# basilevh/tcow

Measured on AMD Instinct MI355X. Metric: train clips/sec (T=30, 240x320), higher is better.
Workload: dtype bf16; 1 GPU; TCOW Seeker train step: T=30 240x320 patch16, 12-layer divided space-time ViT (D=768), num_queries=3, causal_attention=1, 1 clip/GPU; clips_per_gpu=1, num_queries=3, parallelism=dp1, optimizer=AdamW lr 1e-4, clip 0.3

## Files before the change

include/tcow_hip.h:

```cpp
#ifndef TCOW_HIP_H
#define TCOW_HIP_H

#ifdef __cplusplus
extern "C" {
#endif

#define TCOW_OK 0
#define TCOW_ERR_INVALID_ARG (-1)
#define TCOW_ERR_LAUNCH (-2)
#define TCOW_ERR_UNSUPPORTED (-3)

#define TCOW_F32 0
#define TCOW_BF16 1
#define TCOW_F32X3 2

#define TCOW_ACT_NONE 0
#define TCOW_ACT_GELU 1
#define TCOW_ACT_DGELU 2
#define TCOW_ACT_GELU_DSAVE 3
#define TCOW_ACT_MUL_AUX 4

#define TCOW_ABI_VERSION 11
int tcow_version(void);
const char* tcow_last_error(void);

typedef struct {
    int M, N, K;
    int dtype;
    const void* A; long lda;
    const void* W; long ldw;
    void* C; long ldc; int out_f32;
    const float* bias;
    const float* row_scale;
    const float* resid; long ldr;
    int act;
    void* aux; long ldaux;
    int tile;
    const float* bias2;
    const float* row_scale2;
} tcow_gemm_args;
int tcow_gemm_nt(void* stream, const tcow_gemm_args* args);

int tcow_prof_gemm_begin(int max_launches);
int tcow_prof_gemm_end(double* total_ms, double* total_flops, long* launches);
int tcow_prof_attn_begin(int max_launches);
int tcow_prof_attn_end(double* ms4, double* flops4, double* bytes4, long* launches4);

long tcow_gemm_tn_workspace_bytes(int M, int N, int K);
int tcow_gemm_tn(void* stream, int dtype, int M, int N, int K, const void* dY, long ldy, const void* X,
                 long ldx, float* dW, long lddw, float* bias_grad, int accumulate, void* workspace,
                 long workspace_bytes);

typedef struct {
    int M, N, K;
    const void* dY; long ldy;
    const void* X; long ldx;
    float* dW; long lddw;
    float* bias_grad;
    int accumulate;
} tcow_tn_problem;
long tcow_gemm_tn_grouped_workspace_bytes(int dtype, int n, const tcow_tn_problem* problems);
int tcow_gemm_tn_grouped(void* stream, int dtype, int n, const tcow_tn_problem* problems, void* workspace, long workspace_bytes);
int tcow_gemm_tn_group_max(void);

typedef struct {
    int M, N, K;
    const float* A; long sai, sak;
    const float* B; long sbj, sbk;
    float* C; long ldc;
    int accumulate;
} tcow_sgemm;
int tcow_sgemm_x3_batched(void* stream, int n, const tcow_sgemm* problems);

int tcow_layernorm_fwd(void* stream, int dtype, int rows, int D, const float* x, long ldx, const float* gamma,
                       const float* beta, float eps, void* y, long ldy, float* mean, float* rstd);
long tcow_layernorm_bwd_workspace_bytes(int D);
int tcow_layernorm_bwd(void* stream, int dtype, int rows, int D, const void* dy, long lddy, const float* x, long ldx,
                       const float* mean, const float* rstd, const float* gamma, const float* dres, long lddres,
                       float* dx, long lddx, float* dgamma, float* dbeta, int accumulate, void* workspace,
                       long workspace_bytes, void* dx_cast, long lddx_cast, const float* cast_row_scale,
                       const float* colsum_row_scale, float* colsum_out);
typedef struct {
    const float* part; int parts, D;
    float* dgamma; float* dbeta; float* colsum_out;
    int accumulate;
} tcow_ln_fold_job;
int tcow_layernorm_bwd_parts(int rows, int with_colsum);
int tcow_layernorm_fold(void* stream, int n, const tcow_ln_fold_job* jobs);

typedef struct {
    int B, T, S;
    int D, heads;
    int causal;
    int dtype;
} tcow_attn_shape;
int tcow_attn_temporal_fwd(void* stream, const tcow_attn_shape* shape, const void* qkv, void* out, float* lse);
int tcow_attn_spatial_fwd(void* stream, const tcow_attn_shape* shape, const void* qkv, void* out, float* lse);
long tcow_attn_bwd_workspace_bytes(const tcow_attn_shape* shape);
int tcow_attn_temporal_bwd(void* stream, const tcow_attn_shape* shape, const void* qkv, const void* out,
                           const void* dout, const float* lse, void* dqkv, void* workspace, long workspace_bytes);
int tcow_attn_spatial_bwd(void* stream, const tcow_attn_shape* shape, const void* qkv, const void* out,
                          const void* dout, const float* lse, void* dqkv, void* workspace, long workspace_bytes);

#define TCOW_STREAM_MAX_FRAMES 1024
int tcow_attn_temporal_cached_fwd(void* stream, const tcow_attn_shape* chunk, int T_total, const int* t0_dev, const void* qkv, void* k_cache,
                                  void* v_cache, void* out);
int tcow_cls_stream(void* stream, int B, int c, int S, int D, float* x, float* cls_cache, const int* t0_dev);

int tcow_im2col(void* stream, int dtype, int B, int T, int H, int W, int P, const float* rgb, const float* query,
                int pretrained_norm, void* out);
int tcow_im2col_channels(void* stream, int dtype, int B, int T, int H, int W, int P, int C, const float* src,
                         int normalise, void* out);
int tcow_gather_frames(void* stream, int elem_bytes, int C, int Tv, int H, int W, int Tc, int h, int w, const void* src,
                       const int* frame_idx, const int* src_y, const int* src_x, void* out);
int tcow_resize_aa(void* stream, int C, int Tv, int H, int W, int Tc, int hc, int wc, int oh, int ow, const float* src, const int* frame_idx,
                   const int* ys, const int* xs, const int* ymin, const int* ysize, const float* wy, int ky, const int* xmin, const int* xsize,
                   const float* wx, int kx, float* out);

long tcow_photometric_workspace_bytes(int Tc);
int tcow_photometric(void* stream, int Tv, int H, int W, int Tc, int y0, int x0, int h, int w, const float* src, const int* frame_idx, int n_ops,
                     const int* ops, float brightness, float contrast, float saturation, float hue, int blur, const float* taps, int gray,
                     float* workspace, long workspace_bytes, float* out);

int tcow_embed_fwd(void* stream, int B, int T, int S, int D, float* x, const float* cls, const float* pos,
                   const float* time_embed);
int tcow_embed_bwd(void* stream, int B, int T, int S, int D, const float* g, float* dpos, float* dtime,
                   int accumulate);
int tcow_cls_merge(void* stream, int B, int T, int S, int D, float* x, int mode, int backward);
int tcow_cls_merge_bwd_cast(void* stream, int dtype, int B, int T, int S, int D, float* x, int mode, void* cast_out, long ldc,
                            const float* cast_scale);

int tcow_unpatchify_pool_fwd(void* stream, int dtype, int BT, int Hp, int Wp, int P, int C, int st, const void* pm,
                             float* pooled);
int tcow_unpatchify_pool_bwd(void* stream, int dtype, int BT, int Hp, int Wp, int P, int C, int st,
                             const float* dpooled, void* dpm);
int tcow_upsample_fwd(void* stream, int B, int T, int C, int h, int w, int st, int bilinear, const float* pooled,
                      float* out);
int tcow_upsample_bwd(void* stream, int B, int T, int C, int h, int w, int st, int bilinear, const float* dout,
                      float* dpooled);
#define TCOW_AMAX_SLOTS 64
int tcow_upsample_bwd_amax(void* stream, int B, int T, int C, int h, int w, int st, const float* dout, float* dpooled,
                           unsigned* amax_bits, int n_slots);
int tcow_flags_fwd(void* stream, int BT, int S, int D, int F, const float* x, const float* Wf, const float* bf,
                   float* flags);

int tcow_scale_unless_one(void* stream, float* x, long n, const float* scale);
int tcow_scale_cast(void* stream, int dtype, long rows, int D, const float* src, long ld_src, const float* row_scale,
                    void* dst, long ld_dst);
int tcow_droppath_rows(void* stream, int depth, int B, int T, int S, const float* u, const float* keep_p, const float* mask0, float* out);
int tcow_cast_transpose(void* stream, int dtype, int N, int K, const float* W, void* Wc, void* Wt);
long tcow_cast_desc_bytes(void);
int tcow_cast_transpose_batched(void* stream, int dtype, const void* table, int n, int total_tiles);

long tcow_adamw_chunk_bytes(void);
int tcow_adamw_clip_step(void* stream, const void* chunks, int n_chunks, float lr, float beta1, float beta2, float eps,
                         float weight_decay, int step, float max_norm, float* scratch);
int tcow_adamw_clip_step_scaled(void* stream, const void* chunks, int n_chunks, float lr, float beta1, float beta2, float eps,
                                float weight_decay, int step, float max_norm, float* scratch, const float* grad_inv_scale);
long tcow_adamw_tile_bytes(void);
int tcow_adamw_clip_step_cast(void* stream, const void* chunks, int n_chunks, const void* flat_chunks, int n_flat, const void* tiles, int n_tiles, float lr, float beta1,
                              float beta2, float eps, float weight_decay, int step, float max_norm, float* scratch, const float* grad_inv_scale);

typedef struct {
    long n_frames, frame_len, frames_per_seq;
    const float* logits;  long logits_seq_stride;
    const float* target;  long target_seq_stride;
    const float* pixel_w;
    const float* frame_w;
    int weighted_aot;
    float aot_loss;
    double topk_frac;
    float loss_weight;
    float* loss;
    float* total;
    float* dlogits;  long dlogits_seq_stride;
    void* ws;  size_t ws_bytes;
    int focal;
} tcow_mask_loss_args;
size_t tcow_mask_loss_workspace_bytes(long n_frames, long frame_len);
size_t tcow_mask_loss_workspace_bytes_for(long n_frames, long frame_len, double topk_frac, float aot_loss);
int tcow_mask_loss(void* stream, const tcow_mask_loss_args* args);
int tcow_mask_loss_batch(void* stream, const tcow_mask_loss_args* args, int n);

int tcow_iou_counts(void* stream, const float* logits, const float* target, long n_frames, long frame_len, int* counts);

int tcow_build_masks(void* stream, int B, int Q, int M, int T, long HW, int query_time, const unsigned char* segm,
                     const unsigned char* div_segm, const int* query_idx, const int* front_idx, const int* cont_idx,
                     float* query_mask, float* target_mask, unsigned char* snitch_occl_by_ptr, int* counts);

int tcow_build_query_masks(void* stream, int B, int Q, int K, int M, int T, long HW, int query_time, const unsigned char* segm,
                           const unsigned char* div_segm, const float* occl_fracs, const float* dag, const long long* sel, float front_thres,
                           float front_half_thres, float outer_thres, float occluded_weight, float zero_weight, float has_weight, int* idx_ws,
                           unsigned char* ids, float* flags, float* sel_occl_fracs, float* frame_w, float* query_mask, float* target_mask,
                           unsigned char* snitch_occl_by_ptr, int* counts);

int tcow_iou_means(void* stream, const int* counts, int n_seq, int C, int T, float* mean, int* count);

size_t tcow_snitch_weights_workspace_bytes(long n_frames, int H, int W);
int tcow_snitch_weights(void* stream, long n_seq, int T, int H, int W, const float* target_ch0, long target_seq_stride,
                        const unsigned char* snitch_occl_by_ptr, const float* frame_w, const int* pos_count, int class_balancing,
                        float hard_negative_factor, float* weights, void* ws, size_t ws_bytes);

#ifdef __cplusplus
}
#endif
#endif
```

tcow_amd/_lib.py:

```python
import ctypes
import os

_HERE = os.path.dirname(os.path.abspath(__file__))
LIB_PATH = os.environ.get('TCOW_LIB') or os.path.join(_HERE, 'libtcow_hip.so')
LIB_PATH_FP16 = os.path.join(_HERE, 'libtcow_hip_fp16.so')

TCOW_F32, TCOW_BF16, TCOW_F32X3 = 0, 1, 2
ACT_NONE, ACT_GELU, ACT_DGELU, ACT_GELU_DSAVE, ACT_MUL_AUX = 0, 1, 2, 3, 4


class TcowError(RuntimeError):
    """Raised when a libtcow_hip entry point returns a non-zero status (message from tcow_last_error)."""


class AttnShape(ctypes.Structure):
    _fields_ = [('B', ctypes.c_int), ('T', ctypes.c_int), ('S', ctypes.c_int), ('D', ctypes.c_int),
                ('heads', ctypes.c_int), ('causal', ctypes.c_int), ('dtype', ctypes.c_int)]


class GemmArgs(ctypes.Structure):
    _fields_ = [('M', ctypes.c_int), ('N', ctypes.c_int), ('K', ctypes.c_int), ('dtype', ctypes.c_int),
                ('A', ctypes.c_void_p), ('lda', ctypes.c_long), ('W', ctypes.c_void_p), ('ldw', ctypes.c_long),
                ('C', ctypes.c_void_p), ('ldc', ctypes.c_long), ('out_f32', ctypes.c_int),
                ('bias', ctypes.c_void_p), ('row_scale', ctypes.c_void_p), ('resid', ctypes.c_void_p),
                ('ldr', ctypes.c_long), ('act', ctypes.c_int), ('aux', ctypes.c_void_p), ('ldaux', ctypes.c_long), ('tile', ctypes.c_int),
                ('bias2', ctypes.c_void_p), ('row_scale2', ctypes.c_void_p)]


class SGemm(ctypes.Structure):
    _fields_ = [('M', ctypes.c_int), ('N', ctypes.c_int), ('K', ctypes.c_int),
                ('A', ctypes.c_void_p), ('sai', ctypes.c_long), ('sak', ctypes.c_long),
                ('B', ctypes.c_void_p), ('sbj', ctypes.c_long), ('sbk', ctypes.c_long),
                ('C', ctypes.c_void_p), ('ldc', ctypes.c_long), ('accumulate', ctypes.c_int)]


class TnProblem(ctypes.Structure):
    _fields_ = [('M', ctypes.c_int), ('N', ctypes.c_int), ('K', ctypes.c_int),
                ('dY', ctypes.c_void_p), ('ldy', ctypes.c_long), ('X', ctypes.c_void_p), ('ldx', ctypes.c_long),
                ('dW', ctypes.c_void_p), ('lddw', ctypes.c_long), ('bias_grad', ctypes.c_void_p), ('accumulate', ctypes.c_int)]


class LnFoldJob(ctypes.Structure):
    _fields_ = [('part', ctypes.c_void_p), ('parts', ctypes.c_int), ('D', ctypes.c_int), ('dgamma', ctypes.c_void_p), ('dbeta', ctypes.c_void_p),
                ('colsum_out', ctypes.c_void_p), ('accumulate', ctypes.c_int)]


class MaskLossArgs(ctypes.Structure):
    _fields_ = [('n_frames', ctypes.c_long), ('frame_len', ctypes.c_long), ('frames_per_seq', ctypes.c_long),
                ('logits', ctypes.c_void_p), ('logits_seq_stride', ctypes.c_long),
                ('target', ctypes.c_void_p), ('target_seq_stride', ctypes.c_long),
                ('pixel_w', ctypes.c_void_p), ('frame_w', ctypes.c_void_p),
                ('weighted_aot', ctypes.c_int), ('aot_loss', ctypes.c_float), ('topk_frac', ctypes.c_double),
                ('loss_weight', ctypes.c_float), ('loss', ctypes.c_void_p), ('total', ctypes.c_void_p),
                ('dlogits', ctypes.c_void_p), ('dlogits_seq_stride', ctypes.c_long),
                ('ws', ctypes.c_void_p), ('ws_bytes', ctypes.c_size_t), ('focal', ctypes.c_int)]


_libs = {}

_vp, _i, _l, _f = ctypes.c_void_p, ctypes.c_int, ctypes.c_long, ctypes.c_float
_ash = ctypes.POINTER(AttnShape)
SIGNATURES = {
    'tcow_version': (_i, []),
    'tcow_last_error': (ctypes.c_char_p, []),
    'tcow_gemm_nt': (_i, [_vp, ctypes.POINTER(GemmArgs)]),
    'tcow_prof_gemm_begin': (_i, [_i]),
    'tcow_prof_gemm_end': (_i, [ctypes.POINTER(ctypes.c_double), ctypes.POINTER(ctypes.c_double), ctypes.POINTER(ctypes.c_long)]),
    'tcow_prof_attn_begin': (_i, [_i]),
    'tcow_prof_attn_end': (_i, [_vp, _vp, _vp, _vp]),
    'tcow_gemm_tn_workspace_bytes': (_l, [_i, _i, _i]),
    'tcow_gemm_tn': (_i, [_vp, _i, _i, _i, _i, _vp, _l, _vp, _l, _vp, _l, _vp, _i, _vp, _l]),
    'tcow_gemm_tn_grouped_workspace_bytes': (_l, [_i, _i, _vp]),
    'tcow_gemm_tn_grouped': (_i, [_vp, _i, _i, _vp, _vp, _l]),
    'tcow_gemm_tn_group_max': (_i, []),
    'tcow_sgemm_x3_batched': (_i, [_vp, _i, _vp]),
    'tcow_layernorm_fwd': (_i, [_vp, _i, _i, _i, _vp, _l, _vp, _vp, _f, _vp, _l, _vp, _vp]),
    'tcow_layernorm_bwd_workspace_bytes': (_l, [_i]),
    'tcow_layernorm_bwd': (_i, [_vp, _i, _i, _i, _vp, _l, _vp, _l, _vp, _vp, _vp, _vp, _l, _vp, _l, _vp, _vp, _i, _vp, _l, _vp, _l, _vp, _vp, _vp]),
    'tcow_layernorm_bwd_parts': (_i, [_i, _i]),
    'tcow_layernorm_fold': (_i, [_vp, _i, _vp]),
    'tcow_attn_temporal_fwd': (_i, [_vp, _ash, _vp, _vp, _vp]),
    'tcow_attn_spatial_fwd': (_i, [_vp, _ash, _vp, _vp, _vp]),
    'tcow_attn_bwd_workspace_bytes': (_l, [_ash]),
    'tcow_attn_temporal_bwd': (_i, [_vp, _ash, _vp, _vp, _vp, _vp, _vp, _vp, _l]),
    'tcow_attn_spatial_bwd': (_i, [_vp, _ash, _vp, _vp, _vp, _vp, _vp, _vp, _l]),
    'tcow_attn_temporal_cached_fwd': (_i, [_vp, _ash, _i, _vp, _vp, _vp, _vp, _vp]),
    'tcow_cls_stream': (_i, [_vp, _i, _i, _i, _i, _vp, _vp, _vp]),
    'tcow_im2col': (_i, [_vp, _i, _i, _i, _i, _i, _i, _vp, _vp, _i, _vp]),
    'tcow_gather_frames': (_i, [_vp, _i, _i, _i, _i, _i, _i, _i, _i, _vp, _vp, _vp, _vp, _vp]),
    'tcow_resize_aa': (_i, [_vp, _i, _i, _i, _i, _i, _i, _i, _i, _i, _vp, _vp, _vp, _vp, _vp, _vp, _vp, _i, _vp, _vp, _vp, _i, _vp]),
    'tcow_photometric_workspace_bytes': (_l, [_i]),
    'tcow_photometric': (_i, [_vp, _i, _i, _i, _i, _i, _i, _i, _i, _vp, _vp, _i, ctypes.POINTER(ctypes.c_int), _f, _f, _f, _f, _i, ctypes.POINTER(ctypes.c_float), _i,
                         _vp, _l, _vp]),
    'tcow_im2col_channels': (_i, [_vp, _i, _i, _i, _i, _i, _i, _i, _vp, _i, _vp]),
    'tcow_embed_fwd': (_i, [_vp, _i, _i, _i, _i, _vp, _vp, _vp, _vp]),
    'tcow_embed_bwd': (_i, [_vp, _i, _i, _i, _i, _vp, _vp, _vp, _i]),
    'tcow_cls_merge': (_i, [_vp, _i, _i, _i, _i, _vp, _i, _i]),
    'tcow_cls_merge_bwd_cast': (_i, [_vp, _i, _i, _i, _i, _i, _vp, _i, _vp, _l, _vp]),
    'tcow_unpatchify_pool_fwd': (_i, [_vp, _i, _i, _i, _i, _i, _i, _i, _vp, _vp]),
    'tcow_unpatchify_pool_bwd': (_i, [_vp, _i, _i, _i, _i, _i, _i, _i, _vp, _vp]),
    'tcow_upsample_fwd': (_i, [_vp, _i, _i, _i, _i, _i, _i, _i, _vp, _vp]),
    'tcow_upsample_bwd': (_i, [_vp, _i, _i, _i, _i, _i, _i, _i, _vp, _vp]),
    'tcow_upsample_bwd_amax': (_i, [_vp, _i, _i, _i, _i, _i, _i, _vp, _vp, _vp, _i]),
    'tcow_flags_fwd': (_i, [_vp, _i, _i, _i, _i, _vp, _vp, _vp, _vp]),
    'tcow_droppath_rows': (_i, [_vp, _i, _i, _i, _i, _vp, _vp, _vp, _vp]),
    'tcow_scale_cast': (_i, [_vp, _i, _l, _i, _vp, _l, _vp, _vp, _l]),
    'tcow_scale_unless_one': (_i, [_vp, _vp, _l, _vp]),
    'tcow_cast_transpose': (_i, [_vp, _i, _i, _i, _vp, _vp, _vp]),
    'tcow_cast_desc_bytes': (_l, []),
    'tcow_cast_transpose_batched': (_i, [_vp, _i, _vp, _i, _i]),
    'tcow_adamw_chunk_bytes': (_l, []),
    'tcow_adamw_clip_step': (_i, [_vp, _vp, _i, _f, _f, _f, _f, _f, _i, _f, _vp]),
    'tcow_adamw_clip_step_scaled': (_i, [_vp, _vp, _i, _f, _f, _f, _f, _f, _i, _f, _vp, _vp]),
    'tcow_adamw_tile_bytes': (_l, []),
    'tcow_adamw_clip_step_cast': (_i, [_vp, _vp, _i, _vp, _i, _vp, _i, _f, _f, _f, _f, _f, _i, _f, _vp, _vp]),
    'tcow_mask_loss_workspace_bytes': (ctypes.c_size_t, [_l, _l]),
    'tcow_mask_loss_workspace_bytes_for': (ctypes.c_size_t, [_l, _l, ctypes.c_double, _f]),
    'tcow_mask_loss': (_i, [_vp, ctypes.POINTER(MaskLossArgs)]),
    'tcow_mask_loss_batch': (_i, [_vp, ctypes.POINTER(MaskLossArgs), _i]),
    'tcow_iou_counts': (_i, [_vp, _vp, _vp, _l, _l, _vp]),
    'tcow_build_masks': (_i, [_vp, _i, _i, _i, _i, _l, _i, _vp, _vp, _vp, _vp, _vp, _vp, _vp, _vp, _vp]),
    'tcow_build_query_masks': (_i, [_vp, _i, _i, _i, _i, _i, _l, _i, _vp, _vp, _vp, _vp, _vp, _f, _f, _f, _f, _f, _f, _vp, _vp, _vp, _vp, _vp, _vp, _vp, _vp, _vp]),
    'tcow_iou_means': (_i, [_vp, _vp, _i, _i, _i, _vp, _vp]),
    'tcow_snitch_weights_workspace_bytes': (ctypes.c_size_t, [_l, _i, _i]),
    'tcow_snitch_weights': (_i, [_vp, _l, _i, _i, _i, _vp, _l, _vp, _vp, _vp, _i, _f, _vp, _vp, ctypes.c_size_t]),
}


ABI_VERSION = 11


def _declare(L, tolerant=False):
    for name, (res, args) in SIGNATURES.items():
        if tolerant and not hasattr(L, name):
            continue
        fn = getattr(L, name)
        fn.restype = res
        fn.argtypes = args



def lib(fmt='bf16'):
    L = _libs.get(fmt)
    if L is None:
        path = LIB_PATH if fmt == 'bf16' else LIB_PATH_FP16
        if not os.path.exists(path):
            raise TcowError(f'{path} not found: build it with `make` (or __graft_entry__.build()); '
                            'the Seeker HIP path has no fallback')
        import torch
        L = ctypes.CDLL(path)
        L.tcow_last_error.restype = ctypes.c_char_p
        L.tcow_version.restype = ctypes.c_int
        if L.tcow_version() != ABI_VERSION and not (fmt == 'bf16' and os.environ.get('TCOW_LIB')):
            raise TcowError(f'{path} reports ABI version {L.tcow_version()}, this host code was written against {ABI_VERSION} (include/tcow_hip.h): rebuild with `make`')
        _declare(L, tolerant=(fmt == 'bf16' and bool(os.environ.get('TCOW_LIB'))))
        _libs[fmt] = L
    return L


def check(rc, what='', L=None):
    if rc != 0:
        raise TcowError(f'{what} failed (status {rc}): {(L or lib()).tcow_last_error().decode()}')
```

tcow_amd/csrc/common.h:

```cpp
#pragma once
#include <hip/hip_runtime.h>
#include <stdint.h>

#include "../../include/tcow_hip.h"

#ifdef TCOW_FP16
typedef _Float16 tcow_h16;
#define TCOW_MFMA_32x32x16_H16 __builtin_amdgcn_mfma_f32_32x32x16_f16
#define TCOW_MFMA_32x32x16_H16_ASM "v_mfma_f32_32x32x16_f16"
#else
typedef __bf16 tcow_h16;
#define TCOW_MFMA_32x32x16_H16 __builtin_amdgcn_mfma_f32_32x32x16_bf16
#define TCOW_MFMA_32x32x16_H16_ASM "v_mfma_f32_32x32x16_bf16"
#endif
typedef __attribute__((ext_vector_type(8))) tcow_h16 bf16x8;
typedef __attribute__((ext_vector_type(4))) tcow_h16 bf16x4;
typedef __attribute__((ext_vector_type(2))) tcow_h16 bf16x2;
typedef __attribute__((ext_vector_type(16))) float f32x16;
typedef __attribute__((ext_vector_type(4))) float f32x4;
typedef __attribute__((ext_vector_type(2))) float f32x2;
typedef __attribute__((ext_vector_type(4))) short s16x4;
typedef uint16_t bf16_t;

#define LDS_PTR(T) __attribute__((address_space(3))) T*
#define GLB_PTR(T) __attribute__((address_space(1))) T*

void tcow_set_error(const char* fmt, ...);
#define TCOW_CHECK_ARG(cond, ...)                 \
    do {                                          \
        if (!(cond)) {                            \
            tcow_set_error(__VA_ARGS__);          \
            return TCOW_ERR_INVALID_ARG;          \
        }                                         \
    } while (0)
#define TCOW_CHECK_LAUNCH()                                                        \
    do {                                                                           \
        hipError_t e__ = hipGetLastError();                                        \
        if (e__ != hipSuccess) {                                                   \
            tcow_set_error("%s: launch failed: %s", __func__, hipGetErrorString(e__)); \
            return TCOW_ERR_LAUNCH;                                                \
        }                                                                          \
    } while (0)

__device__ __forceinline__ float bf2f(bf16_t h) {
#ifdef TCOW_FP16
    return (float)__builtin_bit_cast(_Float16, h);
#else
    return __builtin_bit_cast(float, ((uint32_t)h) << 16);
#endif
}
__device__ __forceinline__ bf16_t f2bf(float f) { return __builtin_bit_cast(bf16_t, (tcow_h16)f); }
__device__ __forceinline__ uint32_t pack_bf2(float lo, float hi) {
    f32x2 v = {lo, hi};
    bf16x2 b = __builtin_convertvector(v, bf16x2);
    return __builtin_bit_cast(uint32_t, b);
}
#ifdef TCOW_FP16
__device__ __forceinline__ float bflo(uint32_t u) { return (float)__builtin_bit_cast(_Float16, (uint16_t)(u & 0xffffu)); }
__device__ __forceinline__ float bfhi(uint32_t u) { return (float)__builtin_bit_cast(_Float16, (uint16_t)(u >> 16)); }
#else
__device__ __forceinline__ float bflo(uint32_t u) { return __builtin_bit_cast(float, u << 16); }
__device__ __forceinline__ float bfhi(uint32_t u) { return __builtin_bit_cast(float, u & 0xffff0000u); }
#endif

template <typename T> struct Elem;
template <> struct Elem<float> {
    static __device__ __forceinline__ float ld(const float* p) { return *p; }
    static __device__ __forceinline__ void st(float* p, float v) { *p = v; }
};
template <> struct Elem<bf16_t> {
    static __device__ __forceinline__ float ld(const bf16_t* p) { return bf2f(*p); }
    static __device__ __forceinline__ void st(bf16_t* p, float v) { *p = f2bf(v); }
};

__device__ __forceinline__ float4 ld4(const float* p) { return *reinterpret_cast<const float4*>(p); }
__device__ __forceinline__ float4 ld4(const bf16_t* p) {
    uint2 u = *reinterpret_cast<const uint2*>(p);
    return make_float4(bflo(u.x), bfhi(u.x), bflo(u.y), bfhi(u.y));
}
__device__ __forceinline__ void st4(float* p, float4 v) { *reinterpret_cast<float4*>(p) = v; }
__device__ __forceinline__ void st4(bf16_t* p, float4 v) {
    uint2 u; u.x = pack_bf2(v.x, v.y); u.y = pack_bf2(v.z, v.w);
    *reinterpret_cast<uint2*>(p) = u;
}

typedef uint32_t tcow_u32x4 __attribute__((ext_vector_type(4)));
template <bool NT> __device__ __forceinline__ void st16c(void* p, uint4 w) {
    if constexpr (NT) __builtin_nontemporal_store((tcow_u32x4){w.x, w.y, w.z, w.w}, reinterpret_cast<tcow_u32x4*>(p)); else *reinterpret_cast<uint4*>(p) = w;
}
template <bool NT> __device__ __forceinline__ uint4 ld16c(const void* p) {
    if constexpr (NT) { const tcow_u32x4 v = __builtin_nontemporal_load(reinterpret_cast<const tcow_u32x4*>(p)); return make_uint4(v[0], v[1], v[2], v[3]); } else return *reinterpret_cast<const uint4*>(p);
}

__device__ __forceinline__ float gelu_erf(float x) { return 0.5f * x * (1.0f + erff(x * 0.70710678118654752440f)); }
__device__ __forceinline__ float gelu_erf_grad(float x) {
    const float cdf = 0.5f * (1.0f + erff(x * 0.70710678118654752440f));
    const float pdf = 0.39894228040143267794f * __expf(-0.5f * x * x);
    return cdf + x * pdf;
}

__device__ __forceinline__ float wave_sum(float v) {
#pragma unroll
    for (int o = 32; o > 0; o >>= 1) v += __shfl_xor(v, o, 64);
    return v;
}
__device__ __forceinline__ float wave_max(float v) {
#pragma unroll
    for (int o = 32; o > 0; o >>= 1) v = fmaxf(v, __shfl_xor(v, o, 64));
    return v;
}

__host__ __device__ __forceinline__ constexpr int crow32(int r, int hi) { return (r & 3) + 8 * (r >> 2) + 4 * hi; }

void tcow_ensure_lds(const void* kernel, int bytes);

static inline int cdiv(long a, long b) { return (int)((a + b - 1) / b); }
```

tcow_amd/csrc/elementwise.hip:

```cpp
#include "common.h"

namespace {

template <typename T>
__global__ void im2col_kernel(int B, int T_, int H, int W, int P, int Crgb, int Cq, const float* __restrict__ rgb, const float* __restrict__ qm, int norm,
                              T* __restrict__ out) {
    const int Hp = H / P, Wp = W / P, N = Hp * Wp, S = N + 1, C = Crgb + Cq;
    const int Kc = C * P * P, q4 = Kc / 4;
    const long total = (long)B * T_ * S * q4;
    for (long i = blockIdx.x * (long)blockDim.x + threadIdx.x; i < total; i += (long)gridDim.x * blockDim.x) {
        const long row = i / q4; const int k = (int)(i - row * q4) * 4;
        const int s = (int)(row % S); const long bt = row / S; const int t = (int)(bt % T_); const int b = (int)(bt / T_);
        float4 v = make_float4(0.f, 0.f, 0.f, 0.f);
        if (s > 0) {
            const int n = s - 1, hp = n / Wp, wp = n - hp * Wp;
            const int c = k / (P * P), rem = k - c * P * P, py = rem / P, px = rem - py * P;
            const int y = hp * P + py, x = wp * P + px;
            if (c < Crgb) {
                v = ld4(rgb + ((((size_t)b * Crgb + c) * T_ + t) * H + y) * W + x);
                if (norm) { v.x = (v.x - 0.45f) / 0.225f; v.y = (v.y - 0.45f) / 0.225f; v.z = (v.z - 0.45f) / 0.225f; v.w = (v.w - 0.45f) / 0.225f; }
            } else {
                v = ld4(qm + ((((size_t)b * Cq + (c - Crgb)) * T_ + t) * H + y) * W + x);
            }
        }
        st4(out + row * Kc + k, v);
    }
}

template <typename T>
__global__ void gather_frames_kernel(int C, int Tv, int H, int W, int Tc, int h, int w, const T* __restrict__ src, const int* __restrict__ frame_idx,
                                     const int* __restrict__ src_y, const int* __restrict__ src_x, T* __restrict__ out) {
    const long total = (long)C * Tc * h * w;
    for (long i = blockIdx.x * (long)blockDim.x + threadIdx.x; i < total; i += (long)gridDim.x * blockDim.x) {
        const int x = (int)(i % w); long r = i / w; const int y = (int)(r % h); r /= h; const int t = (int)(r % Tc); const int c = (int)(r / Tc);
        out[i] = src[(((size_t)c * Tv + frame_idx[t]) * H + src_y[y]) * W + src_x[x]];
    }
}

__global__ void resize_aa_kernel(int C, int Tv, int H, int W, int Tc, int oh, int ow, const float* __restrict__ src, const int* __restrict__ frame_idx,
                                 const int* __restrict__ ys, const int* __restrict__ xs, const int* __restrict__ ymin, const int* __restrict__ ysize,
                                 const float* __restrict__ wy, int ky, const int* __restrict__ xmin, const int* __restrict__ xsize, const float* __restrict__ wx, int kx,
                                 float* __restrict__ out) {
    const long total = (long)C * Tc * oh * ow;
    for (long i = blockIdx.x * (long)blockDim.x + threadIdx.x; i < total; i += (long)gridDim.x * blockDim.x) {
        const int X = (int)(i % ow); long r = i / ow; const int Y = (int)(r % oh); r /= oh; const int t = (int)(r % Tc); const int c = (int)(r / Tc);
        const float* plane = src + ((size_t)c * Tv + frame_idx[t]) * H * W;
        const int x0 = xmin[X], nx = xsize[X], y0 = ymin[Y], ny = ysize[Y];
        float acc = 0.f;
        for (int j = 0; j < ny; ++j) {
            const float* row = plane + (size_t)ys[y0 + j] * W;
            float h = 0.f;
            for (int k = 0; k < nx; ++k) h += wx[(size_t)X * kx + k] * row[xs[x0 + k]];
            acc += wy[(size_t)Y * ky + j] * h;
        }
        out[i] = acc;
    }
}

__global__ void embed_fwd_kernel(int B, int T_, int S, int D, float* __restrict__ x, const float* __restrict__ cls, const float* __restrict__ pos,
                                 const float* __restrict__ time) {
    const int d4 = D / 4;
    const long total = (long)B * T_ * S * d4;
    for (long i = blockIdx.x * (long)blockDim.x + threadIdx.x; i < total; i += (long)gridDim.x * blockDim.x) {
        const long row = i / d4; const int c = (int)(i - row * d4) * 4;
        const int s = (int)(row % S); const int t = (int)((row / S) % T_);
        const float4 p = ld4(pos + (size_t)s * D + c);
        float4 o;
        if (s == 0) { const float4 cv = ld4(cls + c); o = make_float4(cv.x + p.x, cv.y + p.y, cv.z + p.z, cv.w + p.w); }
        else {
            const float4 v = ld4(x + row * D + c), te = ld4(time + (size_t)t * D + c);
            o = make_float4(v.x + p.x + te.x, v.y + p.y + te.y, v.z + p.z + te.z, v.w + p.w + te.w);
        }
        st4(x + row * D + c, o);
    }
}
__global__ __launch_bounds__(256) void embed_bwd_pos_kernel(int B, int T_, int S, int D, const float* __restrict__ g, float* __restrict__ dpos, int accumulate) {
    __shared__ float4 red[256];
    const int d4 = D / 4, s = blockIdx.x, q = blockIdx.y * 64 + (threadIdx.x & 63), part = threadIdx.x >> 6, BT = B * T_;
    float4 a = make_float4(0.f, 0.f, 0.f, 0.f);
    if (q < d4) {
        const float* src = g + (size_t)s * D + q * 4;
        const size_t fs = (size_t)S * D;
        int bt = part;
        for (; bt + 20 < BT; bt += 24) {
            float4 v[6];
#pragma unroll
            for (int u = 0; u < 6; ++u) v[u] = ld4(src + (size_t)(bt + 4 * u) * fs);
#pragma unroll
            for (int u = 0; u < 6; ++u) { a.x += v[u].x; a.y += v[u].y; a.z += v[u].z; a.w += v[u].w; }
        }
        for (; bt < BT; bt += 4) { const float4 v = ld4(src + (size_t)bt * fs); a.x += v.x; a.y += v.y; a.z += v.z; a.w += v.w; }
    }
    red[threadIdx.x] = a;
    __syncthreads();
    if (part == 0 && q < d4) {
#pragma unroll
        for (int p = 1; p < 4; ++p) { const float4 v = red[p * 64 + threadIdx.x]; a.x += v.x; a.y += v.y; a.z += v.z; a.w += v.w; }
        float* o = dpos + (size_t)s * D + q * 4;
        if (accumulate) { const float4 p = ld4(o); a.x += p.x; a.y += p.y; a.z += p.z; a.w += p.w; }
        st4(o, a);
    }
}
__global__ __launch_bounds__(256) void embed_bwd_time_kernel(int B, int T_, int S, int D, const float* __restrict__ g, float* __restrict__ dtime, int accumulate) {
    __shared__ float4 red[256];
    const int t = blockIdx.x, cq = blockIdx.y * 16 + (threadIdx.x & 15), part = threadIdx.x >> 4;
    const int d4 = D / 4;
    float4 a = make_float4(0.f, 0.f, 0.f, 0.f);
    if (cq < d4) {
        for (int b = 0; b < B; ++b)
            for (int s = 1 + part; s < S; s += 16) {
                const float4 v = ld4(g + (((size_t)b * T_ + t) * S + s) * D + cq * 4); a.x += v.x; a.y += v.y; a.z += v.z; a.w += v.w;
            }
    }
    red[threadIdx.x] = a;
    __syncthreads();
    if (part == 0 && cq < d4) {
        for (int p = 1; p < 16; ++p) { const float4 v = red[p * 16 + (threadIdx.x & 15)]; a.x += v.x; a.y += v.y; a.z += v.z; a.w += v.w; }
        float* o = dtime + (size_t)t * D + cq * 4;
        if (accumulate) { const float4 p = ld4(o); a.x += p.x; a.y += p.y; a.z += p.z; a.w += p.w; }
        st4(o, a);
    }
}

__device__ __forceinline__ float4 sum_frames(const float* base, size_t fs, int T_) {
    float4 a = make_float4(0.f, 0.f, 0.f, 0.f);
    for (int t0 = 0; t0 < T_; t0 += 8) {
        float4 v[8];
#pragma unroll
        for (int u = 0; u < 8; ++u) v[u] = t0 + u < T_ ? ld4(base + (t0 + u) * fs) : make_float4(0.f, 0.f, 0.f, 0.f);
#pragma unroll
        for (int u = 0; u < 8; ++u) { a.x += v[u].x; a.y += v[u].y; a.z += v[u].z; a.w += v[u].w; }
    }
    return a;
}
template <typename CT>
__global__ void cls_merge_kernel(int B, int T_, int S, int D, float* __restrict__ x, int mode, int backward, CT* __restrict__ cast_out, long ldc,
                                 const float* __restrict__ cast_scale) {
    const int d4 = D / 4;
    const long i = blockIdx.x * (long)blockDim.x + threadIdx.x;
    if (i >= (long)B * d4) return;
    const int b = (int)(i / d4), c = (int)(i - (long)b * d4) * 4;
    float* base = x + (size_t)b * T_ * S * D + c;
    const size_t fs = (size_t)S * D;
    if (!backward) {
        float4 a;
        if (mode == 1) a = ld4(base);
        else {
            a = sum_frames(base, fs, T_);
            const float inv = 1.0f / (float)T_; a.x *= inv; a.y *= inv; a.z *= inv; a.w *= inv;
        }
        for (int t = 0; t < T_; ++t) st4(base + t * fs, a);
    } else {
        float4 a = sum_frames(base, fs, T_);
        if (mode == 1) {
            st4(base, a);
            const float4 z = make_float4(0.f, 0.f, 0.f, 0.f);
            for (int t = 1; t < T_; ++t) st4(base + t * fs, z);
        } else {
            const float inv = 1.0f / (float)T_; a.x *= inv; a.y *= inv; a.z *= inv; a.w *= inv;
            for (int t = 0; t < T_; ++t) st4(base + t * fs, a);
        }
        if (cast_out) {
            for (int t0 = 0; t0 < T_; t0 += 8) {
                float cs[8];
#pragma unroll
                for (int u = 0; u < 8; ++u) cs[u] = (cast_scale && t0 + u < T_ && !(mode == 1 && t0 + u > 0)) ? cast_scale[((long)b * T_ + t0 + u) * S] : 1.0f;
#pragma unroll
                for (int u = 0; u < 8; ++u) {
                    const int t = t0 + u;
                    if (t < T_) {
                        const float4 v = (mode == 1 && t > 0) ? make_float4(0.f, 0.f, 0.f, 0.f) : make_float4(a.x * cs[u], a.y * cs[u], a.z * cs[u], a.w * cs[u]);
                        st4(cast_out + ((long)b * T_ + t) * S * ldc + c, v);
                    }
                }
            }
        }
    }
}

template <typename T>
__global__ void unpatchify_pool_fwd_kernel(int BT, int Hp, int Wp, int P, int C, int st, const T* __restrict__ pm, float* __restrict__ pooled) {
    const int S = Hp * Wp + 1, Ps = P / st, Ho = Hp * Ps, Wo = Wp * Ps, K = C * P * P;
    const long total = (long)BT * C * Ho * Wo;
    const float inv = 1.0f / (float)(st * st);
    for (long i = blockIdx.x * (long)blockDim.x + threadIdx.x; i < total; i += (long)gridDim.x * blockDim.x) {
        const int X = (int)(i % Wo); const int Y = (int)((i / Wo) % Ho); const int c = (int)((i / ((long)Wo * Ho)) % C); const long bt = i / ((long)Wo * Ho * C);
        const int hp = Y / Ps, py0 = (Y - hp * Ps) * st, wp = X / Ps, px0 = (X - wp * Ps) * st;
        const T* src = pm + ((size_t)bt * S + 1 + hp * Wp + wp) * K + (size_t)c * P * P;
        float a = 0.f;
        for (int dy = 0; dy < st; ++dy)
            for (int dx = 0; dx < st; ++dx) a += Elem<T>::ld(src + (py0 + dy) * P + px0 + dx);
        pooled[i] = a * inv;
    }
}
template <typename T>
__global__ __launch_bounds__(256) void unpatchify_pool4_fwd_kernel(int BT, int Hp, int Wp, int P, int C, const T* __restrict__ pm, float* __restrict__ pooled) {
    const int S = Hp * Wp + 1, Ps = P / 4, Ho = Hp * Ps, Wo = Wp * Ps, K = C * P * P, P8 = P / 8;
    const int per_tok = C * Ps * P8;
    const long total = (long)BT * (S - 1) * per_tok;
    for (long i = blockIdx.x * (long)blockDim.x + threadIdx.x; i < total; i += (long)gridDim.x * blockDim.x) {
        const int tok = (int)(i / per_tok), r = (int)(i - (long)tok * per_tok);
        const int piece = r % P8, yb = (r / P8) % Ps, c = r / (P8 * Ps);
        const int bt = tok / (S - 1), n = tok - bt * (S - 1), hp = n / Wp, wp = n - hp * Wp;
        const T* src = pm + ((size_t)bt * S + 1 + n) * K + (size_t)c * P * P + (4 * yb) * P + piece * 8;
        float a0 = 0.f, a1 = 0.f;
#pragma unroll
        for (int dy = 0; dy < 4; ++dy) {
            const float4 u = ld4(src + dy * P), v = ld4(src + dy * P + 4);
            a0 += (u.x + u.y) + (u.z + u.w); a1 += (v.x + v.y) + (v.z + v.w);
        }
        float* o = pooled + (((size_t)bt * C + c) * Ho + hp * Ps + yb) * Wo + wp * Ps + piece * 2;
        *reinterpret_cast<float2*>(o) = make_float2(a0 * 0.0625f, a1 * 0.0625f);
    }
}

template <typename T>
__global__ void unpatchify_pool_bwd_kernel(int BT, int Hp, int Wp, int P, int C, int st, const float* __restrict__ dpooled, T* __restrict__ dpm) {
    const int S = Hp * Wp + 1, Ps = P / st, Ho = Hp * Ps, Wo = Wp * Ps, K = C * P * P;
    const long total = (long)BT * S * K;
    const float inv = 1.0f / (float)(st * st);
    for (long i = blockIdx.x * (long)blockDim.x + threadIdx.x; i < total; i += (long)gridDim.x * blockDim.x) {
        const int k = (int)(i % K); const long row = i / K; const int s = (int)(row % S); const long bt = row / S;
        float v = 0.f;
        if (s > 0) {
            const int n = s - 1, hp = n / Wp, wp = n - hp * Wp;
            const int c = k / (P * P), rem = k - c * P * P, py = rem / P, px = rem - py * P;
            const int Y = hp * Ps + py / st, X = wp * Ps + px / st;
            v = dpooled[(((size_t)bt * C + c) * Ho + Y) * Wo + X] * inv;
        }
        Elem<T>::st(dpm + i, v);
    }
}

template <typename T>
__global__ __launch_bounds__(256) void unpatchify_pool_bwd8_kernel(int rows, int Hp, int Wp, int P, int C, int st, const float* __restrict__ dpooled, T* __restrict__ dpm) {
    const int S = Hp * Wp + 1, Ps = P / st, Ho = Hp * Ps, Wo = Wp * Ps, K = C * P * P, K8 = K >> 3;
    const float inv = 1.0f / (float)(st * st);
    const long total = (long)rows * K8;
    for (long i = blockIdx.x * (long)blockDim.x + threadIdx.x; i < total; i += (long)gridDim.x * blockDim.x) {
        const int row = (int)(i / K8), k = (int)(i - (long)row * K8) * 8;
        const int bt = row / S, s = row - bt * S;
        float v[8] = {0.f, 0.f, 0.f, 0.f, 0.f, 0.f, 0.f, 0.f};
        if (s > 0) {
            const int n = s - 1, hp = n / Wp, wp = n - hp * Wp;
            const int c = k / (P * P), rem = k - c * P * P, py = rem / P, px = rem - py * P;
            const float* src = dpooled + (((size_t)bt * C + c) * Ho + hp * Ps + py / st) * Wo + wp * Ps;
#pragma unroll
            for (int e = 0; e < 8; ++e) v[e] = src[(px + e) / st] * inv;
        }
        T* dst = dpm + (size_t)row * K + k;
        st4(dst, make_float4(v[0], v[1], v[2], v[3]));
        st4(dst + 4, make_float4(v[4], v[5], v[6], v[7]));
    }
}

__device__ __forceinline__ void bil_src(int dst, int in, int out, int& i0, int& i1, float& w0, float& w1) {
    const float scale = (out > 1) ? (float)(in - 1) / (float)(out - 1) : 0.f;
    const float src = scale * (float)dst;
    i0 = (int)src; if (i0 > in - 1) i0 = in - 1;
    i1 = i0 + ((i0 < in - 1) ? 1 : 0);
    w1 = src - (float)i0; w0 = 1.0f - w1;
}
__global__ void upsample_fwd_kernel(int B, int T_, int C, int h, int w, int st, int bilinear, const float* __restrict__ pooled, float* __restrict__ out) {
    const int H = h * st, W = w * st;
    const int f = blockIdx.y;
    const int t = f % T_, bc = f / T_, c = bc % C, b = bc / C;
    const float* src = pooled + (((size_t)(b * T_ + t)) * C + c) * h * w;
    float* dst = out + (size_t)f * H * W;
    const int Wq = (W + 3) / 4;
    for (int i = blockIdx.x * blockDim.x + threadIdx.x; i < H * Wq; i += gridDim.x * blockDim.x) {
        const int y = i / Wq, x0q = (i - y * Wq) * 4;
        float v[4];
        int y0, y1; float wy0, wy1;
        if (bilinear) bil_src(y, h, H, y0, y1, wy0, wy1);
#pragma unroll
        for (int e = 0; e < 4; ++e) {
            const int x = x0q + e < W ? x0q + e : W - 1;
            if (bilinear) {
                int x0, x1; float wx0, wx1;
                bil_src(x, w, W, x0, x1, wx0, wx1);
                v[e] = wy0 * (wx0 * src[y0 * w + x0] + wx1 * src[y0 * w + x1]) + wy1 * (wx0 * src[y1 * w + x0] + wx1 * src[y1 * w + x1]);
            } else {
                v[e] = src[(y / st) * w + (x / st)];
            }
        }
        float* o = dst + (size_t)y * W + x0q;
        if ((W & 3) == 0) st4(o, make_float4(v[0], v[1], v[2], v[3]));
        else for (int e = 0; e < 4 && x0q + e < W; ++e) o[e] = v[e];
    }
}
__global__ void upsample_bwd_kernel(int B, int T_, int C, int h, int w, int st, int bilinear, const float* __restrict__ dout, float* __restrict__ dpooled,
                                    unsigned* __restrict__ amax_bits) {
    const int H = h * st, W = w * st;
    const long total = (long)B * T_ * C * h * w;
    float amax = 0.f;
    for (long i = blockIdx.x * (long)blockDim.x + threadIdx.x; i < total; i += (long)gridDim.x * blockDim.x) {
        const int X = (int)(i % w); const int Y = (int)((i / w) % h); const int c = (int)((i / ((long)w * h)) % C); const long bt = i / ((long)w * h * C);
        const int b = (int)(bt / T_), t = (int)(bt - (long)b * T_);
        const float* g = dout + (((size_t)b * C + c) * T_ + t) * H * W;
        float a = 0.f;
        if (bilinear && st == 4 && h > 4 && w > 4) {
            float wx[12];
            const int xa = 4 * X - 4, ya = 4 * Y - 4;
#pragma unroll
            for (int e = 0; e < 12; ++e) {
                const int x = xa + e;
                wx[e] = 0.f;
                if (x >= 0 && x < W) { int x0, x1; float wx0, wx1; bil_src(x, w, W, x0, x1, wx0, wx1); if (x0 == X) wx[e] += wx0; if (x1 == X) wx[e] += wx1; }
            }
            for (int e = 0; e < 12; ++e) {
                const int y = ya + e;
                if (y < 0 || y >= H) continue;
                int y0, y1; float wy0, wy1; bil_src(y, h, H, y0, y1, wy0, wy1);
                float wy = 0.f; if (y0 == Y) wy += wy0; if (y1 == Y) wy += wy1;
                if (wy == 0.f) continue;
                const float* row = g + (size_t)y * W + xa;
                float r = 0.f;
#pragma unroll
                for (int q = 0; q < 3; ++q) {
                    if (xa + 4 * q >= 0 && xa + 4 * q + 3 < W) {
                        const float4 v = ld4(row + 4 * q);
                        r += wx[4 * q] * v.x + wx[4 * q + 1] * v.y + wx[4 * q + 2] * v.z + wx[4 * q + 3] * v.w;
                        if (amax_bits && q == 1) amax = fmaxf(amax, fmaxf(fmaxf(fabsf(v.x), fabsf(v.y)), fmaxf(fabsf(v.z), fabsf(v.w))));
                    }
                }
                a += wy * r;
            }
        } else if (bilinear) {
            const float isy = (h > 1) ? (float)(H - 1) / (float)(h - 1) : 0.f, isx = (w > 1) ? (float)(W - 1) / (float)(w - 1) : 0.f;
            int ylo = (int)((float)(Y - 1) * isy) - 1, yhi = (int)((float)(Y + 1) * isy) + 2; if (ylo < 0) ylo = 0; if (yhi > H - 1) yhi = H - 1;
            int xlo = (int)((float)(X - 1) * isx) - 1, xhi = (int)((float)(X + 1) * isx) + 2; if (xlo < 0) xlo = 0; if (xhi > W - 1) xhi = W - 1;
            if (h <= 1) { ylo = 0; yhi = H - 1; }
            if (w <= 1) { xlo = 0; xhi = W - 1; }
            for (int y = ylo; y <= yhi; ++y) {
                int y0, y1; float wy0, wy1; bil_src(y, h, H, y0, y1, wy0, wy1);
                float wy = 0.f; if (y0 == Y) wy += wy0; if (y1 == Y) wy += wy1;
                if (wy == 0.f) continue;
                for (int x = xlo; x <= xhi; ++x) {
                    int x0, x1; float wx0, wx1; bil_src(x, w, W, x0, x1, wx0, wx1);
                    float wx = 0.f; if (x0 == X) wx += wx0; if (x1 == X) wx += wx1;
                    if (wx != 0.f) a += wy * wx * g[(size_t)y * W + x];
                }
            }
        } else {
            for (int dy = 0; dy < st; ++dy)
                for (int dx = 0; dx < st; ++dx) a += g[(size_t)(Y * st + dy) * W + X * st + dx];
        }
        dpooled[i] = a;
    }
    if (amax_bits) {
        __shared__ float wmax[4];
        for (int o = 32; o > 0; o >>= 1) amax = fmaxf(amax, __shfl_xor(amax, o, 64));
        if ((threadIdx.x & 63) == 0) wmax[threadIdx.x >> 6] = amax;
        __syncthreads();
        if (threadIdx.x == 0) {
            const float m = fmaxf(fmaxf(wmax[0], wmax[1]), fmaxf(wmax[2], wmax[3]));
            if (m > 0.f) atomicMax(amax_bits + (blockIdx.x & (TCOW_AMAX_SLOTS - 1)), __builtin_bit_cast(unsigned, m));
        }
    }
}

__global__ __launch_bounds__(1024) void flags_fwd_kernel(int S, int D, int F, const float* __restrict__ x, const float* __restrict__ Wf, const float* __restrict__ bf,
                                                         float* __restrict__ flags) {
    extern __shared__ float4 part[];
    const int bt = blockIdx.x;
    const int D4 = D >> 2;
    const int G = 1024 / D4 > 0 ? 1024 / D4 : 1;
    const float4* xb = reinterpret_cast<const float4*>(x + (size_t)bt * S * D);
    for (int idx = threadIdx.x; idx < G * D4; idx += 1024) {
        const int g = idx / D4, c = idx - g * D4;
        float4 a = make_float4(0.f, 0.f, 0.f, 0.f);
#pragma unroll 4
        for (int s = 1 + g; s < S; s += G) {
            const float4 v = xb[(size_t)s * D4 + c];
            a.x += v.x; a.y += v.y; a.z += v.z; a.w += v.w;
        }
        part[idx] = a;
    }
    __syncthreads();
    const float inv = 1.0f / (float)(S - 1);
    for (int c = threadIdx.x; c < D4; c += 1024) {
        float4 a = part[c];
        for (int g = 1; g < G; ++g) { const float4 v = part[g * D4 + c]; a.x += v.x; a.y += v.y; a.z += v.z; a.w += v.w; }
        part[c] = make_float4(a.x * inv, a.y * inv, a.z * inv, a.w * inv);
    }
    __syncthreads();
    const float* mean = reinterpret_cast<const float*>(part);
    const int wave = threadIdx.x >> 6, lane = threadIdx.x & 63;
    for (int f = wave; f < F; f += 16) {
        float a = 0.f;
        for (int d = lane; d < D; d += 64) a += mean[d] * Wf[(size_t)f * D + d];
        a = wave_sum(a);
        if (lane == 0) flags[(size_t)bt * F + f] = a + bf[f];
    }
}

struct CastDesc { const float* W; void* Wc; void* Wt; int N, K, tile_begin, tile; };
template <typename T>
__global__ __launch_bounds__(256) void cast_transpose_batched_kernel(const CastDesc* __restrict__ tab, int n) {
    __shared__ float tile[64][65];
    int lo = 0, hi = n - 1;
    const int b = blockIdx.x;
    while (lo < hi) { const int mid = (lo + hi + 1) >> 1; if (tab[mid].tile_begin <= b) lo = mid; else hi = mid - 1; }
    const CastDesc d = tab[lo];
    T* Wc = reinterpret_cast<T*>(d.Wc); T* Wt = reinterpret_cast<T*>(d.Wt);
    if (d.tile == 64) {
        const int t = b - d.tile_begin, tiles_k = d.K >> 6;
        const int n0 = (t / tiles_k) * 64, k0 = (t - (t / tiles_k) * tiles_k) * 64;
        const int c4 = (threadIdx.x & 15) * 4, r0 = threadIdx.x >> 4;
#pragma unroll
        for (int i = 0; i < 4; ++i) {
            const int r = r0 + 16 * i;
            const float4 v = ld4(d.W + (size_t)(n0 + r) * d.K + k0 + c4);
            if (Wc) st4(Wc + (size_t)(n0 + r) * d.K + k0 + c4, v);
            tile[r][c4] = v.x; tile[r][c4 + 1] = v.y; tile[r][c4 + 2] = v.z; tile[r][c4 + 3] = v.w;
        }
        __syncthreads();
        if (Wt) {
#pragma unroll
            for (int i = 0; i < 4; ++i) {
                const int k = r0 + 16 * i;
                st4(Wt + (size_t)(k0 + k) * d.N + n0 + c4, make_float4(tile[c4][k], tile[c4 + 1][k], tile[c4 + 2][k], tile[c4 + 3][k]));
            }
        }
        return;
    }
    const int t = b - d.tile_begin, tiles_k = (d.K + 31) / 32;
    const int n0 = (t / tiles_k) * 32, k0 = (t - (t / tiles_k) * tiles_k) * 32;
    const int tx = threadIdx.x & 31, ty = threadIdx.x >> 5;
    for (int r = ty; r < 32; r += 8) {
        const int nn = n0 + r, k = k0 + tx;
        float v = 0.f;
        if (nn < d.N && k < d.K) { v = d.W[(size_t)nn * d.K + k]; if (Wc) Elem<T>::st(Wc + (size_t)nn * d.K + k, v); }
        tile[r][tx] = v;
    }
    __syncthreads();
    if (Wt)
        for (int r = ty; r < 32; r += 8) {
            const int k = k0 + r, nn = n0 + tx;
            if (k < d.K && nn < d.N) Elem<T>::st(Wt + (size_t)k * d.N + nn, tile[tx][r]);
        }
}

template <typename T>
__global__ void scale_cast_kernel(long rows, int D, const float* __restrict__ src, long lds_, const float* __restrict__ row_scale, T* __restrict__ dst, long ldd) {
    const int d4 = D / 4;
    const long total = rows * d4;
    for (long i = blockIdx.x * (long)blockDim.x + threadIdx.x; i < total; i += (long)gridDim.x * blockDim.x) {
        const long row = i / d4; const int c = (int)(i - row * d4) * 4;
        float4 v = ld4(src + row * lds_ + c);
        if (row_scale) { const float s = row_scale[row]; v.x *= s; v.y *= s; v.z *= s; v.w *= s; }
        st4(dst + row * ldd + c, v);
    }
}
template <typename T>
__global__ __launch_bounds__(256) void cast_transpose_kernel(int N, int K, const float* __restrict__ Wsrc, T* __restrict__ Wc, T* __restrict__ Wt) {
    __shared__ float tile[32][33];
    const int n0 = blockIdx.y * 32, k0 = blockIdx.x * 32;
    const int tx = threadIdx.x & 31, ty = threadIdx.x >> 5;
    for (int r = ty; r < 32; r += 8) {
        const int n = n0 + r, k = k0 + tx;
        float v = 0.f;
        if (n < N && k < K) { v = Wsrc[(size_t)n * K + k]; if (Wc) Elem<T>::st(Wc + (size_t)n * K + k, v); }
        tile[r][tx] = v;
    }
    __syncthreads();
    if (Wt)
        for (int r = ty; r < 32; r += 8) {
            const int k = k0 + r, n = n0 + tx;
            if (n < N && k < K) Elem<T>::st(Wt + (size_t)k * N + n, tile[tx][r]);
        }
}

}

static inline int gs_blocks(long total, int per_block = 256) { long b = (total + per_block - 1) / per_block; return (int)(b > 4096 ? 4096 : (b < 1 ? 1 : b)); }

__global__ void __launch_bounds__(256) droppath_rows_kernel(int depth, int B, int T, int S, const float* __restrict__ u, const float* __restrict__ keep_p,
                                                            const float* __restrict__ mask0, float* __restrict__ out) {
    const long M = (long)B * T * S, n = (long)depth * M;
    const int N = S - 1, per = B * N + B * T + B;
    for (long i = blockIdx.x * 256L + threadIdx.x; i < n; i += (long)gridDim.x * 256) {
        const int l = (int)(i / M); const long r = i - (long)l * M;
        const int b = (int)(r / ((long)T * S)), ts = (int)(r - (long)b * T * S), t = ts / S, sp = ts - t * S;
        const float kp = keep_p[l];
        const float* ul = u + (long)l * per;
        const float st = sp == 0 ? 1.0f : floorf(ul[b * N + sp - 1] + kp) / kp;
        const float ss = floorf(ul[B * N + b * T + t] + kp) / kp;
        const float sm = floorf(ul[B * N + B * T + b] + kp) / kp;
        out[i] = st; out[n + i] = ss; out[2 * n + i] = sm; out[3 * n + i] = st * mask0[r];
    }
}

extern "C" {

int tcow_im2col(void* stream, int dtype, int B, int T_, int H, int W, int P, const float* rgb, const float* query, int pretrained_norm, void* out) {
    TCOW_CHECK_ARG(B > 0 && T_ > 0 && P > 0 && P % 4 == 0 && H % P == 0 && W % P == 0, "tcow_im2col: bad geometry B=%d T=%d H=%d W=%d P=%d", B, T_, H, W, P);
    TCOW_CHECK_ARG(rgb && query && out, "tcow_im2col: null pointer");
    const long total = (long)B * T_ * ((H / P) * (W / P) + 1) * (4 * P * P / 4);
    if (dtype == TCOW_BF16) hipLaunchKernelGGL(im2col_kernel<bf16_t>, dim3(gs_blocks(total)), dim3(256), 0, (hipStream_t)stream, B, T_, H, W, P, 3, 1, rgb, query, pretrained_norm, (bf16_t*)out);
    else if (dtype == TCOW_F32) hipLaunchKernelGGL(im2col_kernel<float>, dim3(gs_blocks(total)), dim3(256), 0, (hipStream_t)stream, B, T_, H, W, P, 3, 1, rgb, query, pretrained_norm, (float*)out);
    else { tcow_set_error("tcow_im2col: unknown dtype %d", dtype); return TCOW_ERR_INVALID_ARG; }
    TCOW_CHECK_LAUNCH();
    return TCOW_OK;
}

int tcow_gather_frames(void* stream, int elem_bytes, int C, int Tv, int H, int W, int Tc, int h, int w, const void* src, const int* frame_idx,
                       const int* src_y, const int* src_x, void* out) {
    TCOW_CHECK_ARG(C > 0 && Tv > 0 && H > 0 && W > 0 && Tc > 0 && h > 0 && w > 0 && src && frame_idx && src_y && src_x && out, "tcow_gather_frames: bad arguments");
    TCOW_CHECK_ARG(elem_bytes == 1 || elem_bytes == 4, "tcow_gather_frames: elem_bytes must be 1 or 4 (got %d)", elem_bytes);
    const long total = (long)C * Tc * h * w;
    if (elem_bytes == 1) hipLaunchKernelGGL(gather_frames_kernel<uint8_t>, dim3(gs_blocks(total)), dim3(256), 0, (hipStream_t)stream, C, Tv, H, W, Tc, h, w, (const uint8_t*)src, frame_idx, src_y, src_x, (uint8_t*)out);
    else hipLaunchKernelGGL(gather_frames_kernel<uint32_t>, dim3(gs_blocks(total)), dim3(256), 0, (hipStream_t)stream, C, Tv, H, W, Tc, h, w, (const uint32_t*)src, frame_idx, src_y, src_x, (uint32_t*)out);
    TCOW_CHECK_LAUNCH();
    return TCOW_OK;
}

int tcow_resize_aa(void* stream, int C, int Tv, int H, int W, int Tc, int hc, int wc, int oh, int ow, const float* src, const int* frame_idx, const int* ys, const int* xs,
                   const int* ymin, const int* ysize, const float* wy, int ky, const int* xmin, const int* xsize, const float* wx, int kx, float* out) {
    TCOW_CHECK_ARG(C > 0 && Tv > 0 && H > 0 && W > 0 && Tc > 0 && hc > 0 && wc > 0 && oh > 0 && ow > 0 && ky > 0 && kx > 0, "tcow_resize_aa: bad geometry");
    TCOW_CHECK_ARG(src && frame_idx && ys && xs && ymin && ysize && wy && xmin && xsize && wx && out, "tcow_resize_aa: null pointer");
    const long total = (long)C * Tc * oh * ow;
    hipLaunchKernelGGL(resize_aa_kernel, dim3(gs_blocks(total)), dim3(256), 0, (hipStream_t)stream, C, Tv, H, W, Tc, oh, ow, src, frame_idx, ys, xs, ymin, ysize, wy, ky, xmin, xsize,
                       wx, kx, out);
    TCOW_CHECK_LAUNCH();
    return TCOW_OK;
}

int tcow_im2col_channels(void* stream, int dtype, int B, int T_, int H, int W, int P, int C, const float* src, int normalise, void* out) {
    TCOW_CHECK_ARG(B > 0 && T_ > 0 && C > 0 && P > 0 && P % 4 == 0 && H % P == 0 && W % P == 0, "tcow_im2col_channels: bad geometry B=%d T=%d H=%d W=%d P=%d C=%d", B, T_, H, W, P, C);
    TCOW_CHECK_ARG(src && out, "tcow_im2col_channels: null pointer");
    const long total = (long)B * T_ * ((H / P) * (W / P) + 1) * (C * P * P / 4);
    if (dtype == TCOW_BF16) hipLaunchKernelGGL(im2col_kernel<bf16_t>, dim3(gs_blocks(total)), dim3(256), 0, (hipStream_t)stream, B, T_, H, W, P, C, 0, src, src, normalise, (bf16_t*)out);
    else if (dtype == TCOW_F32) hipLaunchKernelGGL(im2col_kernel<float>, dim3(gs_blocks(total)), dim3(256), 0, (hipStream_t)stream, B, T_, H, W, P, C, 0, src, src, normalise, (float*)out);
    else { tcow_set_error("tcow_im2col_channels: unknown dtype %d", dtype); return TCOW_ERR_INVALID_ARG; }
    TCOW_CHECK_LAUNCH();
    return TCOW_OK;
}

int tcow_embed_fwd(void* stream, int B, int T_, int S, int D, float* x, const float* cls, const float* pos, const float* time_embed) {
    TCOW_CHECK_ARG(B > 0 && T_ > 0 && S > 1 && D % 4 == 0 && x && cls && pos && time_embed, "tcow_embed_fwd: bad arguments");
    hipLaunchKernelGGL(embed_fwd_kernel, dim3(gs_blocks((long)B * T_ * S * D / 4)), dim3(256), 0, (hipStream_t)stream, B, T_, S, D, x, cls, pos, time_embed);
    TCOW_CHECK_LAUNCH();
    return TCOW_OK;
}

int tcow_embed_bwd(void* stream, int B, int T_, int S, int D, const float* g, float* dpos, float* dtime, int accumulate) {
    TCOW_CHECK_ARG(B > 0 && T_ > 0 && S > 1 && D % 4 == 0 && g && dpos && dtime, "tcow_embed_bwd: bad arguments");
    hipLaunchKernelGGL(embed_bwd_pos_kernel, dim3(S, cdiv(D / 4, 64)), dim3(256), 0, (hipStream_t)stream, B, T_, S, D, g, dpos, accumulate);
    TCOW_CHECK_LAUNCH();
    hipLaunchKernelGGL(embed_bwd_time_kernel, dim3(T_, cdiv(D / 4, 16)), dim3(256), 0, (hipStream_t)stream, B, T_, S, D, g, dtime, accumulate);
    TCOW_CHECK_LAUNCH();
    return TCOW_OK;
}

int tcow_cls_merge(void* stream, int B, int T_, int S, int D, float* x, int mode, int backward) {
    TCOW_CHECK_ARG(B > 0 && T_ > 0 && S > 1 && D % 4 == 0 && x && (mode == 0 || mode == 1), "tcow_cls_merge: bad arguments");
    hipLaunchKernelGGL(cls_merge_kernel<float>, dim3(cdiv((long)B * D / 4, 64)), dim3(64), 0, (hipStream_t)stream, B, T_, S, D, x, mode, backward, (float*)nullptr, 0L, (const float*)nullptr);
    TCOW_CHECK_LAUNCH();
    return TCOW_OK;
}

int tcow_cls_merge_bwd_cast(void* stream, int dtype, int B, int T_, int S, int D, float* x, int mode, void* cast_out, long ldc, const float* cast_scale) {
    TCOW_CHECK_ARG(B > 0 && T_ > 0 && S > 1 && D % 4 == 0 && x && (mode == 0 || mode == 1) && cast_out && ldc % 4 == 0, "tcow_cls_merge_bwd_cast: bad arguments");
    const dim3 grid(cdiv((long)B * D / 4, 64));
    if (dtype == TCOW_BF16) hipLaunchKernelGGL(cls_merge_kernel<bf16_t>, grid, dim3(64), 0, (hipStream_t)stream, B, T_, S, D, x, mode, 1, (bf16_t*)cast_out, ldc, cast_scale);
    else if (dtype == TCOW_F32) hipLaunchKernelGGL(cls_merge_kernel<float>, grid, dim3(64), 0, (hipStream_t)stream, B, T_, S, D, x, mode, 1, (float*)cast_out, ldc, cast_scale);
    else { tcow_set_error("tcow_cls_merge_bwd_cast: unknown dtype %d", dtype); return TCOW_ERR_INVALID_ARG; }
    TCOW_CHECK_LAUNCH();
    return TCOW_OK;
}

int tcow_unpatchify_pool_fwd(void* stream, int dtype, int BT, int Hp, int Wp, int P, int C, int st, const void* pm, float* pooled) {
    TCOW_CHECK_ARG(BT > 0 && Hp > 0 && Wp > 0 && P > 0 && C > 0 && st > 0 && P % st == 0 && pm && pooled, "tcow_unpatchify_pool_fwd: bad arguments");
    const long total = (long)BT * C * Hp * Wp * (P / st) * (P / st);
    if (st == 4 && P % 8 == 0 && ((P / 4) * Wp) % 2 == 0 && (dtype == TCOW_BF16 || dtype == TCOW_F32)) {
        const long nthr = (long)BT * Hp * Wp * C * (P / 4) * (P / 8);
        if (dtype == TCOW_BF16) hipLaunchKernelGGL(unpatchify_pool4_fwd_kernel<bf16_t>, dim3(gs_blocks(nthr)), dim3(256), 0, (hipStream_t)stream, BT, Hp, Wp, P, C, (const bf16_t*)pm, pooled);
        else hipLaunchKernelGGL(unpatchify_pool4_fwd_kernel<float>, dim3(gs_blocks(nthr)), dim3(256), 0, (hipStream_t)stream, BT, Hp, Wp, P, C, (const float*)pm, pooled);
        TCOW_CHECK_LAUNCH();
        return TCOW_OK;
    }
    if (dtype == TCOW_BF16) hipLaunchKernelGGL(unpatchify_pool_fwd_kernel<bf16_t>, dim3(gs_blocks(total)), dim3(256), 0, (hipStream_t)stream, BT, Hp, Wp, P, C, st, (const bf16_t*)pm, pooled);
    else if (dtype == TCOW_F32) hipLaunchKernelGGL(unpatchify_pool_fwd_kernel<float>, dim3(gs_blocks(total)), dim3(256), 0, (hipStream_t)stream, BT, Hp, Wp, P, C, st, (const float*)pm, pooled);
    else { tcow_set_error("tcow_unpatchify_pool_fwd: unknown dtype %d", dtype); return TCOW_ERR_INVALID_ARG; }
    TCOW_CHECK_LAUNCH();
    return TCOW_OK;
}

int tcow_unpatchify_pool_bwd(void* stream, int dtype, int BT, int Hp, int Wp, int P, int C, int st, const float* dpooled, void* dpm) {
    TCOW_CHECK_ARG(BT > 0 && Hp > 0 && Wp > 0 && P > 0 && C > 0 && st > 0 && P % st == 0 && dpooled && dpm, "tcow_unpatchify_pool_bwd: bad arguments");
    const long total = (long)BT * (Hp * Wp + 1) * C * P * P;
    if (P % 8 == 0 && (dtype == TCOW_BF16 || dtype == TCOW_F32) && (reinterpret_cast<uintptr_t>(dpm) & 15) == 0) {
        const int rows = BT * (Hp * Wp + 1);
        if (dtype == TCOW_BF16) hipLaunchKernelGGL(unpatchify_pool_bwd8_kernel<bf16_t>, dim3(gs_blocks(total / 8)), dim3(256), 0, (hipStream_t)stream, rows, Hp, Wp, P, C, st, dpooled, (bf16_t*)dpm);
        else hipLaunchKernelGGL(unpatchify_pool_bwd8_kernel<float>, dim3(gs_blocks(total / 8)), dim3(256), 0, (hipStream_t)stream, rows, Hp, Wp, P, C, st, dpooled, (float*)dpm);
        TCOW_CHECK_LAUNCH();
        return TCOW_OK;
    }
    if (dtype == TCOW_BF16) hipLaunchKernelGGL(unpatchify_pool_bwd_kernel<bf16_t>, dim3(gs_blocks(total)), dim3(256), 0, (hipStream_t)stream, BT, Hp, Wp, P, C, st, dpooled, (bf16_t*)dpm);
    else if (dtype == TCOW_F32) hipLaunchKernelGGL(unpatchify_pool_bwd_kernel<float>, dim3(gs_blocks(total)), dim3(256), 0, (hipStream_t)stream, BT, Hp, Wp, P, C, st, dpooled, (float*)dpm);
    else { tcow_set_error("tcow_unpatchify_pool_bwd: unknown dtype %d", dtype); return TCOW_ERR_INVALID_ARG; }
    TCOW_CHECK_LAUNCH();
    return TCOW_OK;
}

int tcow_upsample_fwd(void* stream, int B, int T_, int C, int h, int w, int st, int bilinear, const float* pooled, float* out) {
    TCOW_CHECK_ARG(B > 0 && T_ > 0 && C > 0 && h > 0 && w > 0 && st > 0 && pooled && out, "tcow_upsample_fwd: bad arguments");
    TCOW_CHECK_ARG((long)B * C * T_ < 65536, "tcow_upsample_fwd: too many frames for one call");
    { const int per = h * st * ((w * st + 3) / 4); int gx = cdiv(per, 256); if (gx > 64) gx = 64;
      hipLaunchKernelGGL(upsample_fwd_kernel, dim3(gx, B * C * T_), dim3(256), 0, (hipStream_t)stream, B, T_, C, h, w, st, bilinear, pooled, out); }
    TCOW_CHECK_LAUNCH();
    return TCOW_OK;
}

int tcow_upsample_bwd(void* stream, int B, int T_, int C, int h, int w, int st, int bilinear, const float* dout, float* dpooled) {
    TCOW_CHECK_ARG(B > 0 && T_ > 0 && C > 0 && h > 0 && w > 0 && st > 0 && dout && dpooled, "tcow_upsample_bwd: bad arguments");
    hipLaunchKernelGGL(upsample_bwd_kernel, dim3(gs_blocks((long)B * C * T_ * h * w)), dim3(256), 0, (hipStream_t)stream, B, T_, C, h, w, st, bilinear, dout, dpooled, (unsigned*)nullptr);
    TCOW_CHECK_LAUNCH();
    return TCOW_OK;
}

int tcow_upsample_bwd_amax(void* stream, int B, int T_, int C, int h, int w, int st, const float* dout, float* dpooled, unsigned* amax_bits, int n_slots) {
    TCOW_CHECK_ARG(B > 0 && T_ > 0 && C > 0 && h > 4 && w > 4 && st == 4 && dout && dpooled && amax_bits, "tcow_upsample_bwd_amax: bilinear stride 4 with h, w > 4 only");
    TCOW_CHECK_ARG(n_slots == TCOW_AMAX_SLOTS, "tcow_upsample_bwd_amax: amax_bits must hold TCOW_AMAX_SLOTS = %d words (got %d)", TCOW_AMAX_SLOTS, n_slots);
    hipLaunchKernelGGL(upsample_bwd_kernel, dim3(gs_blocks((long)B * C * T_ * h * w)), dim3(256), 0, (hipStream_t)stream, B, T_, C, h, w, st, 1, dout, dpooled, amax_bits);
    TCOW_CHECK_LAUNCH();
    return TCOW_OK;
}

int tcow_flags_fwd(void* stream, int BT, int S, int D, int F, const float* x, const float* Wf, const float* bf, float* flags) {
    TCOW_CHECK_ARG(BT > 0 && S > 1 && D > 0 && F > 0 && x && Wf && bf && flags, "tcow_flags_fwd: bad arguments");
    TCOW_CHECK_ARG(D % 4 == 0, "tcow_flags_fwd: D %d must be a multiple of 4", D);
    const int D4 = D / 4, G = 1024 / D4 > 0 ? 1024 / D4 : 1;
    hipLaunchKernelGGL(flags_fwd_kernel, dim3(BT), dim3(1024), (size_t)G * D4 * 16, (hipStream_t)stream, S, D, F, x, Wf, bf, flags);
    TCOW_CHECK_LAUNCH();
    return TCOW_OK;
}

__global__ __launch_bounds__(256) void scale_unless_one_kernel(float* __restrict__ x, long n4, long n, const float* __restrict__ scale) {
    const float s = scale[0];
    if (s == 1.0f) return;
    for (long i = blockIdx.x * (long)blockDim.x + threadIdx.x; i < n4; i += (long)gridDim.x * blockDim.x) {
        float4 v = ld4(x + i * 4); v.x *= s; v.y *= s; v.z *= s; v.w *= s; st4(x + i * 4, v);
    }
    if (blockIdx.x == 0 && threadIdx.x < n - n4 * 4) x[n4 * 4 + threadIdx.x] *= s;
}

int tcow_scale_unless_one(void* stream, float* x, long n, const float* scale) {
    TCOW_CHECK_ARG(x && scale && n > 0 && ((uintptr_t)x & 15) == 0, "tcow_scale_unless_one: bad arguments");
    hipLaunchKernelGGL(scale_unless_one_kernel, dim3(gs_blocks(n / 4 + 1)), dim3(256), 0, (hipStream_t)stream, x, n / 4, n, scale);
    TCOW_CHECK_LAUNCH();
    return TCOW_OK;
}

int tcow_scale_cast(void* stream, int dtype, long rows, int D, const float* src, long ld_src, const float* row_scale, void* dst, long ld_dst) {
    TCOW_CHECK_ARG(rows > 0 && D > 0 && D % 4 == 0 && src && dst && ld_src % 4 == 0 && ld_dst % 4 == 0, "tcow_scale_cast: bad arguments");
    if (dtype == TCOW_BF16) hipLaunchKernelGGL(scale_cast_kernel<bf16_t>, dim3(gs_blocks(rows * D / 4)), dim3(256), 0, (hipStream_t)stream, rows, D, src, ld_src, row_scale, (bf16_t*)dst, ld_dst);
    else if (dtype == TCOW_F32) hipLaunchKernelGGL(scale_cast_kernel<float>, dim3(gs_blocks(rows * D / 4)), dim3(256), 0, (hipStream_t)stream, rows, D, src, ld_src, row_scale, (float*)dst, ld_dst);
    else { tcow_set_error("tcow_scale_cast: unknown dtype %d", dtype); return TCOW_ERR_INVALID_ARG; }
    TCOW_CHECK_LAUNCH();
    return TCOW_OK;
}

int tcow_cast_transpose(void* stream, int dtype, int N, int K, const float* W, void* Wc, void* Wt) {
    TCOW_CHECK_ARG(N > 0 && K > 0 && W && (Wc || Wt), "tcow_cast_transpose: bad arguments");
    const dim3 grid(cdiv(K, 32), cdiv(N, 32));
    if (dtype == TCOW_BF16) hipLaunchKernelGGL(cast_transpose_kernel<bf16_t>, grid, dim3(256), 0, (hipStream_t)stream, N, K, W, (bf16_t*)Wc, (bf16_t*)Wt);
    else if (dtype == TCOW_F32) hipLaunchKernelGGL(cast_transpose_kernel<float>, grid, dim3(256), 0, (hipStream_t)stream, N, K, W, (float*)Wc, (float*)Wt);
    else { tcow_set_error("tcow_cast_transpose: unknown dtype %d", dtype); return TCOW_ERR_INVALID_ARG; }
    TCOW_CHECK_LAUNCH();
    return TCOW_OK;
}

long tcow_cast_desc_bytes(void) { return (long)sizeof(CastDesc); }

int tcow_cast_transpose_batched(void* stream, int dtype, const void* table, int n, int total_tiles) {
    TCOW_CHECK_ARG(table && n > 0 && total_tiles > 0, "tcow_cast_transpose_batched: bad arguments");
    if (dtype == TCOW_BF16) hipLaunchKernelGGL(cast_transpose_batched_kernel<bf16_t>, dim3(total_tiles), dim3(256), 0, (hipStream_t)stream, (const CastDesc*)table, n);
    else if (dtype == TCOW_F32) hipLaunchKernelGGL(cast_transpose_batched_kernel<float>, dim3(total_tiles), dim3(256), 0, (hipStream_t)stream, (const CastDesc*)table, n);
    else { tcow_set_error("tcow_cast_transpose_batched: unknown dtype %d", dtype); return TCOW_ERR_INVALID_ARG; }
    TCOW_CHECK_LAUNCH();
    return TCOW_OK;
}

int tcow_droppath_rows(void* stream, int depth, int B, int T, int S, const float* u, const float* keep_p, const float* mask0, float* out) {
    TCOW_CHECK_ARG(depth > 0 && B > 0 && T > 0 && S > 1 && u && keep_p && mask0 && out, "tcow_droppath_rows: bad arguments");
    const long n = (long)depth * B * T * S;
    hipLaunchKernelGGL(droppath_rows_kernel, dim3(gs_blocks(n)), dim3(256), 0, (hipStream_t)stream, depth, B, T, S, u, keep_p, mask0, out);
    TCOW_CHECK_LAUNCH();
    return TCOW_OK;
}

}
```

tcow_amd/csrc/layernorm.hip:

```cpp
#include <stdlib.h>

#include "common.h"

namespace {

constexpr int LN_MAXV = 8;

template <typename T, int NV, bool FULL>
__global__ __launch_bounds__(256) void ln_fwd_kernel(int rows, int D, const float* __restrict__ x, long ldx, const float* __restrict__ gamma,
                                                     const float* __restrict__ beta, float eps, T* __restrict__ y, long ldy,
                                                     float* __restrict__ mean_out, float* __restrict__ rstd_out) {
    const int lane = threadIdx.x & 63;
    const int nv = D >> 2;
    const int rstep = gridDim.x * 4;
    int row = blockIdx.x * 4 + (threadIdx.x >> 6);
    if (row >= rows) return;
    float4 g[NV], b[NV], nx[NV];
#pragma unroll
    for (int i = 0; i < NV; ++i) {
        const int c = lane + i * 64;
        if (FULL || c < nv) { g[i] = ld4(gamma + c * 4); b[i] = ld4(beta + c * 4); nx[i] = ld4(x + (size_t)row * ldx + c * 4); }
    }
    for (; row < rows; row += rstep) {
        float4 v[NV];
        float s = 0.f;
#pragma unroll
        for (int i = 0; i < NV; ++i) {
            const int c = lane + i * 64;
            if (FULL || c < nv) { v[i] = nx[i]; s += (v[i].x + v[i].y) + (v[i].z + v[i].w); }
        }
        if (row + rstep < rows) {
#pragma unroll
            for (int i = 0; i < NV; ++i) {
                const int c = lane + i * 64;
                if (FULL || c < nv) nx[i] = ld4(x + (size_t)(row + rstep) * ldx + c * 4);
            }
        }
        const float mean = wave_sum(s) / (float)D;
        float q = 0.f;
#pragma unroll
        for (int i = 0; i < NV; ++i) {
            const int c = lane + i * 64;
            if (FULL || c < nv) {
                const float a = v[i].x - mean, bb = v[i].y - mean, cc = v[i].z - mean, d = v[i].w - mean;
                q += (a * a + bb * bb) + (cc * cc + d * d);
            }
        }
        const float rstd = 1.0f / sqrtf(wave_sum(q) / (float)D + eps);
        if (lane == 0) {
            if (mean_out) mean_out[row] = mean;
            if (rstd_out) rstd_out[row] = rstd;
        }
        T* yr = y + (size_t)row * ldy;
#pragma unroll
        for (int i = 0; i < NV; ++i) {
            const int c = lane + i * 64;
            if (FULL || c < nv) {
                float4 o;
                o.x = (v[i].x - mean) * rstd * g[i].x + b[i].x; o.y = (v[i].y - mean) * rstd * g[i].y + b[i].y;
                o.z = (v[i].z - mean) * rstd * g[i].z + b[i].z; o.w = (v[i].w - mean) * rstd * g[i].w + b[i].w;
                st4(yr + c * 4, o);
            }
        }
    }
}

template <typename T, int NV, bool CSUM, bool FULL>
__global__ __launch_bounds__(256) void ln_bwd_kernel(int rows, int D, const T* __restrict__ dy, long lddy, const float* __restrict__ x, long ldx,
                                                     const float* __restrict__ mean, const float* __restrict__ rstd,
                                                     const float* __restrict__ gamma, const float* __restrict__ dres, long lddres,
                                                     float* __restrict__ dx, long lddx, float* __restrict__ part ,
                                                     T* __restrict__ dxc, long lddxc, const float* __restrict__ cscale, const float* __restrict__ sumscale) {
    constexpr int NP = CSUM ? 3 : 2;
    extern __shared__ __attribute__((aligned(16))) float red[];
    const int lane = threadIdx.x & 63, wave = threadIdx.x >> 6;
    const int nv = D >> 2;
    float4 gsum[NV], bsum[NV], gam[NV], csum[CSUM ? NV : 1];
#pragma unroll
    for (int i = 0; i < NV; ++i) {
        gsum[i] = make_float4(0.f, 0.f, 0.f, 0.f); bsum[i] = gsum[i];
        if (CSUM) csum[i] = gsum[i];
        const int c = lane + i * 64;
        gam[i] = (FULL || c < nv) ? ld4(gamma + c * 4) : gsum[i];
    }
    const int rstep = gridDim.x * 4;
    int row = blockIdx.x * 4 + wave;
    float4 xn[NV], dn[NV], rn[NV];
    float mu_n = 0.f, rs_n = 0.f;
    auto fetch = [&](int r) {
        mu_n = mean[r]; rs_n = rstd[r];
#pragma unroll
        for (int i = 0; i < NV; ++i) {
            const int c = lane + i * 64;
            if (FULL || c < nv) {
                {
                    typedef float f4v __attribute__((ext_vector_type(4)));
                    const f4v t = __builtin_nontemporal_load(reinterpret_cast<const f4v*>(x + (size_t)r * ldx + c * 4));
                    xn[i] = make_float4(t[0], t[1], t[2], t[3]);
                }
                dn[i] = ld4(dy + (size_t)r * lddy + c * 4);
            }
        }
        if (dres) {
#pragma unroll
            for (int i = 0; i < NV; ++i) {
                const int c = lane + i * 64;
                if (FULL || c < nv) rn[i] = ld4(dres + (size_t)r * lddres + c * 4);
            }
        }
    };
    if (row < rows) fetch(row);
    for (; row < rows; row += rstep) {
        const float mu = mu_n, rs = rs_n;
        float4 xh[NV], g[NV], rr[NV];
        float s1 = 0.f, s2 = 0.f;
#pragma unroll
        for (int i = 0; i < NV; ++i) {
            const int c = lane + i * 64;
            if (FULL || c < nv) {
                const float4 xv = xn[i], d = dn[i];
                rr[i] = rn[i];
                xh[i] = make_float4((xv.x - mu) * rs, (xv.y - mu) * rs, (xv.z - mu) * rs, (xv.w - mu) * rs);
                g[i] = make_float4(d.x * gam[i].x, d.y * gam[i].y, d.z * gam[i].z, d.w * gam[i].w);
                s1 += (g[i].x + g[i].y) + (g[i].z + g[i].w);
                s2 += (g[i].x * xh[i].x + g[i].y * xh[i].y) + (g[i].z * xh[i].z + g[i].w * xh[i].w);
                gsum[i].x += d.x * xh[i].x; gsum[i].y += d.y * xh[i].y; gsum[i].z += d.z * xh[i].z; gsum[i].w += d.w * xh[i].w;
                bsum[i].x += d.x; bsum[i].y += d.y; bsum[i].z += d.z; bsum[i].w += d.w;
            }
        }
        if (row + rstep < rows) fetch(row + rstep);
        const float m1 = wave_sum(s1) / (float)D, m2 = wave_sum(s2) / (float)D;
        float* dxr = dx + (size_t)row * lddx;
        const float cs_row = (dxc && cscale) ? cscale[row] : 1.0f;
        const float ss_row = (CSUM && sumscale) ? sumscale[row] : 1.0f;
        float4 o[NV];
#pragma unroll
        for (int i = 0; i < NV; ++i)
            o[i] = make_float4(rs * (g[i].x - m1 - xh[i].x * m2), rs * (g[i].y - m1 - xh[i].y * m2), rs * (g[i].z - m1 - xh[i].z * m2), rs * (g[i].w - m1 - xh[i].w * m2));
        if (dres) {
#pragma unroll
            for (int i = 0; i < NV; ++i) { o[i].x += rr[i].x; o[i].y += rr[i].y; o[i].z += rr[i].z; o[i].w += rr[i].w; }
        }
#pragma unroll
        for (int i = 0; i < NV; ++i) {
            const int c = lane + i * 64;
            if (FULL || c < nv) {
                st4(dxr + c * 4, o[i]);
                if (CSUM) { csum[i].x = fmaf(ss_row, o[i].x, csum[i].x); csum[i].y = fmaf(ss_row, o[i].y, csum[i].y); csum[i].z = fmaf(ss_row, o[i].z, csum[i].z); csum[i].w = fmaf(ss_row, o[i].w, csum[i].w); }
            }
        }
        if (dxc) {
            const float cs = cs_row;
#pragma unroll
            for (int i = 0; i < NV; ++i) {
                const int c = lane + i * 64;
                if (FULL || c < nv) st4(dxc + (size_t)row * lddxc + c * 4, make_float4(o[i].x * cs, o[i].y * cs, o[i].z * cs, o[i].w * cs));
            }
        }
    }
    if (!part) return;
#pragma unroll
    for (int qn = 0; qn < NP; ++qn) {
#pragma unroll
        for (int i = 0; i < NV; ++i) {
            const int c = lane + i * 64;
            if (FULL || c < nv) *reinterpret_cast<float4*>(red + (size_t)wave * D + c * 4) = qn == 0 ? gsum[i] : (qn == 1 ? bsum[i] : csum[CSUM ? i : 0]);
        }
        __syncthreads();
        for (int i = threadIdx.x; i < D; i += 256)
            part[((size_t)blockIdx.x * NP + qn) * D + i] = (red[i] + red[D + i]) + (red[2 * D + i] + red[3 * D + i]);
        __syncthreads();
    }
}

}

int tcow_launch_row_reduce2(hipStream_t stream, const float* part, int nrows, long ld, int N1, float* out1, int N2, float* out2, int accumulate);
int tcow_launch_row_reduce_group(hipStream_t stream, int n, const float* const* part, const int* nrows, const long* ld, const int* N1, float* const* out1, const int* N2,
                                 float* const* out2, const int* N3, float* const* out3, const int* accumulate);
int tcow_launch_row_reduce3(hipStream_t stream, const float* part, int nrows, long ld, int N1, float* out1, int N2, float* out2, int N3, float* out3, int accumulate);

static const int kLnBwdBlocks = 768;
static const int kLnBwdBlocksCsum = 512;
static const int kLnFwdBlocks = 4096;

extern "C" {

int tcow_layernorm_fwd(void* stream, int dtype, int rows, int D, const float* x, long ldx, const float* gamma, const float* beta, float eps, void* y,
                       long ldy, float* mean, float* rstd) {
    TCOW_CHECK_ARG(rows > 0 && D > 0 && D % 4 == 0 && D <= 64 * 4 * LN_MAXV, "tcow_layernorm_fwd: D=%d must be a multiple of 4 and <= %d", D, 64 * 4 * LN_MAXV);
    TCOW_CHECK_ARG(x && gamma && beta && y && ldx % 4 == 0 && ldy % 4 == 0, "tcow_layernorm_fwd: bad pointers / strides");
    int fblocks = cdiv(rows, 4); if (fblocks > kLnFwdBlocks) fblocks = kLnFwdBlocks;
    const dim3 grid(fblocks), block(256);
    if (dtype != TCOW_BF16 && dtype != TCOW_F32) { tcow_set_error("tcow_layernorm_fwd: unknown dtype %d", dtype); return TCOW_ERR_INVALID_ARG; }
    const int nvl = (D / 4 + 63) / 64;
#define LN_FWD(NVV, FULLV)                                                                                                                               \
    do {                                                                                                                                          \
        if (dtype == TCOW_BF16) hipLaunchKernelGGL((ln_fwd_kernel<bf16_t, NVV, FULLV>), grid, block, 0, (hipStream_t)stream, rows, D, x, ldx, gamma, beta, eps, (bf16_t*)y, ldy, mean, rstd); \
        else hipLaunchKernelGGL((ln_fwd_kernel<float, NVV, FULLV>), grid, block, 0, (hipStream_t)stream, rows, D, x, ldx, gamma, beta, eps, (float*)y, ldy, mean, rstd); \
    } while (0)
    const bool full = D == 256 * nvl && nvl <= 4;
    if (full) { if (nvl == 1) LN_FWD(1, true); else if (nvl == 2) LN_FWD(2, true); else if (nvl == 3) LN_FWD(3, true); else LN_FWD(4, true); }
    else if (nvl <= 1) LN_FWD(1, false); else if (nvl == 2) LN_FWD(2, false); else if (nvl == 3) LN_FWD(3, false); else if (nvl == 4) LN_FWD(4, false); else LN_FWD(8, false);
#undef LN_FWD
    TCOW_CHECK_LAUNCH();
    return TCOW_OK;
}

long tcow_layernorm_bwd_workspace_bytes(int D) { return (long)kLnBwdBlocks * 3 * D * 4; }

int tcow_layernorm_bwd(void* stream, int dtype, int rows, int D, const void* dy, long lddy, const float* x, long ldx, const float* mean,
                       const float* rstd, const float* gamma, const float* dres, long lddres, float* dx, long lddx, float* dgamma, float* dbeta,
                       int accumulate, void* workspace, long workspace_bytes, void* dx_cast, long lddx_cast, const float* cast_row_scale,
                       const float* colsum_row_scale, float* colsum_out) {
    TCOW_CHECK_ARG(rows > 0 && D > 0 && D % 4 == 0 && D <= 64 * 4 * LN_MAXV, "tcow_layernorm_bwd: bad D=%d", D);
    TCOW_CHECK_ARG(dy && x && mean && rstd && gamma && dx, "tcow_layernorm_bwd: null pointer");
    TCOW_CHECK_ARG(!dx_cast || lddx_cast % 4 == 0, "tcow_layernorm_bwd: dx_cast stride must be a multiple of 4");
    const bool want_param_grads = dgamma != nullptr || dbeta != nullptr;
    TCOW_CHECK_ARG(!want_param_grads || (dgamma && dbeta && workspace && workspace_bytes >= tcow_layernorm_bwd_workspace_bytes(D)),
                   "tcow_layernorm_bwd: parameter gradients need dgamma, dbeta and a workspace of %ld bytes", tcow_layernorm_bwd_workspace_bytes(D));
    TCOW_CHECK_ARG(!colsum_out || want_param_grads, "tcow_layernorm_bwd: colsum_out rides on the parameter-gradient pass (dgamma / dbeta needed)");
    const bool csum = colsum_out != nullptr;
    const int max_blocks = csum ? kLnBwdBlocksCsum : kLnBwdBlocks;
    int blocks = cdiv(rows, 4); if (blocks > max_blocks) blocks = max_blocks;
    float* part = want_param_grads ? (float*)workspace : nullptr;
    const size_t lds = want_param_grads ? (size_t)4 * D * 4 : 0;
    if (dtype != TCOW_BF16 && dtype != TCOW_F32) { tcow_set_error("tcow_layernorm_bwd: unknown dtype %d", dtype); return TCOW_ERR_INVALID_ARG; }
    const int nvl = (D / 4 + 63) / 64;
#define LN_BWD(NVV, FULLV)                                                                                                                               \
    do {                                                                                                                                          \
        if (dtype == TCOW_BF16 && csum) hipLaunchKernelGGL((ln_bwd_kernel<bf16_t, NVV, true, FULLV>), dim3(blocks), dim3(256), lds, (hipStream_t)stream, rows, D, (const bf16_t*)dy, lddy, x, ldx, mean, rstd, gamma, dres, lddres, dx, lddx, part, (bf16_t*)dx_cast, lddx_cast, cast_row_scale, colsum_row_scale); \
        else if (dtype == TCOW_BF16) hipLaunchKernelGGL((ln_bwd_kernel<bf16_t, NVV, false, FULLV>), dim3(blocks), dim3(256), lds, (hipStream_t)stream, rows, D, (const bf16_t*)dy, lddy, x, ldx, mean, rstd, gamma, dres, lddres, dx, lddx, part, (bf16_t*)dx_cast, lddx_cast, cast_row_scale, colsum_row_scale); \
        else if (csum) hipLaunchKernelGGL((ln_bwd_kernel<float, NVV, true, FULLV>), dim3(blocks), dim3(256), lds, (hipStream_t)stream, rows, D, (const float*)dy, lddy, x, ldx, mean, rstd, gamma, dres, lddres, dx, lddx, part, (float*)dx_cast, lddx_cast, cast_row_scale, colsum_row_scale); \
        else hipLaunchKernelGGL((ln_bwd_kernel<float, NVV, false, FULLV>), dim3(blocks), dim3(256), lds, (hipStream_t)stream, rows, D, (const float*)dy, lddy, x, ldx, mean, rstd, gamma, dres, lddres, dx, lddx, part, (float*)dx_cast, lddx_cast, cast_row_scale, colsum_row_scale); \
    } while (0)
    const bool full = D == 256 * nvl && nvl <= 4;
    if (full) { if (nvl == 1) LN_BWD(1, true); else if (nvl == 2) LN_BWD(2, true); else if (nvl == 3) LN_BWD(3, true); else LN_BWD(4, true); }
    else if (nvl <= 1) LN_BWD(1, false); else if (nvl == 2) LN_BWD(2, false); else if (nvl == 3) LN_BWD(3, false); else if (nvl == 4) LN_BWD(4, false); else LN_BWD(8, false);
#undef LN_BWD
    TCOW_CHECK_LAUNCH();
    if (want_param_grads && !(accumulate & 2)) {
        if (csum) return tcow_launch_row_reduce3((hipStream_t)stream, part, blocks, 3L * D, D, dgamma, D, dbeta, D, colsum_out, accumulate & 1);
        return tcow_launch_row_reduce2((hipStream_t)stream, part, blocks, 2L * D, D, dgamma, D, dbeta, accumulate & 1);
    }
    return TCOW_OK;
}

int tcow_layernorm_bwd_parts(int rows, int with_colsum) {
    const int max_blocks = with_colsum ? kLnBwdBlocksCsum : kLnBwdBlocks;
    int blocks = cdiv(rows, 4); if (blocks > max_blocks) blocks = max_blocks;
    return blocks;
}

int tcow_layernorm_fold(void* stream, int n, const tcow_ln_fold_job* jobs) {
    TCOW_CHECK_ARG(n > 0 && n <= 16 && jobs, "tcow_layernorm_fold: 1..16 jobs");
    const float* part[16]; int nrows[16]; long ld[16]; int N1[16], N2[16], N3[16], acc[16]; float* o1[16]; float* o2[16]; float* o3[16];
    for (int i = 0; i < n; ++i) {
        const tcow_ln_fold_job& j = jobs[i];
        TCOW_CHECK_ARG(j.part && j.dgamma && j.dbeta && j.parts > 0 && j.D > 0, "tcow_layernorm_fold: bad job %d", i);
        part[i] = j.part; nrows[i] = j.parts; ld[i] = (j.colsum_out ? 3L : 2L) * j.D; N1[i] = N2[i] = N3[i] = j.D; acc[i] = j.accumulate;
        o1[i] = j.dgamma; o2[i] = j.dbeta; o3[i] = j.colsum_out;
    }
    return tcow_launch_row_reduce_group((hipStream_t)stream, n, part, nrows, ld, N1, o1, N2, o2, N3, o3, acc);
}

}
```

tcow_amd/engine.py:

```python
import os
import torch

from . import ops
from .ops import ACT_GELU, ACT_GELU_DSAVE, ACT_MUL_AUX
from .operands import fold_on


def _layout(module):
    if module.attention_type == 'divided_space_time':
        return 20, dict(tn=0, tqkv=2, tproj=4, tfc=6, n1=8, qkv=10, proj=12, n2=14, fc1=16, fc2=18)
    return 12, dict(n1=0, qkv=2, proj=4, n2=6, fc1=8, fc2=10)


def _joint_rows(module, g, dev):
    def build():
        B, T, S = g['B'], g['T'], g['S']
        r = torch.arange(B * T * S, device=dev).reshape(B, T * S)
        keep = torch.ones(T * S, dtype=torch.bool, device=dev)
        keep[torch.arange(1, T, device=dev) * S] = False
        return r[:, keep].reshape(-1).contiguous()
    return module._operands.constant(('jrows', g['B'], str(dev)), build)


def group_sizes(depth, spec=None):
    if spec is None:
        spec = os.environ.get('TCOW_DDP_GROUP') or ('5,5,2' if depth == 12 else '4')
    want = [max(1, int(x)) for x in str(spec).split(',') if x.strip()] or [4]
    sizes, left, k = [], depth, 0
    while left > 0:
        gs = min(want[min(k, len(want) - 1)], left)
        sizes.append(gs); left -= gs; k += 1
    return sizes


def _row_vectors(module, g, train):
    B, T, S, N = g['B'], g['T'], g['S'], g['N']
    dev = module.vit.pos_embed.device
    def build_mask0():
        m = torch.ones(B, T, S, dtype=torch.float32, device=dev)
        m[:, :, 0] = 0
        return m.reshape(-1).contiguous()
    mask0 = module._operands.constant(('mask0', B, T, str(dev)), build_mask0)
    depth = module.network_depth
    rates = torch.linspace(0, module.drop_path_rate, depth).tolist() if depth > 1 else [0.0]
    scales = []
    forced = module.forced_drop_masks
    joint = module.attention_type != 'divided_space_time'
    if joint:
        for i in range(depth):
            ent = {'t': None, 's': None, 'm': None}
            for kind, name in (('s', 'spatial'), ('m', 'mlp')):
                if forced is not None:
                    if (i, name) in forced:
                        keep, rate = forced[(i, name)]
                        ent[kind] = (keep.to(dev, torch.float32).reshape(B) / (1.0 - rate))[:, None].expand(B, T * S).reshape(-1).contiguous()
                elif train and rates[i] > 0.:
                    keep = (torch.rand(B, device=dev) + (1.0 - rates[i])).floor_()
                    ent[kind] = (keep / (1.0 - rates[i]))[:, None].expand(B, T * S).reshape(-1).contiguous()
            scales.append(ent)
        return mask0, scales
    if forced is None and train and max(rates) > 0.:
        keep_p = module._operands.constant(('keep_p', tuple(rates), str(dev)), lambda: (1.0 - torch.tensor(rates, dtype=torch.float32)).to(dev))
        u = torch.rand(depth, B * N + B * T + B, device=dev)
        if u.is_cuda and N == S - 1:
            from . import ops
            rt, rsp, rml, rt0 = ops.droppath_rows(u, keep_p, mask0, B, T, S)
        else:
            kp = keep_p[:, None]
            sc = (u + kp).floor_() / kp
            kt = sc[:, :B * N].reshape(depth, B, 1, N); ks = sc[:, B * N:B * N + B * T].reshape(depth, B, T, 1); km = sc[:, B * N + B * T:].reshape(depth, B, 1)
            rt = torch.ones(depth, B, T, S, dtype=torch.float32, device=dev)
            rt[:, :, :, 1:] = kt
            rt = rt.reshape(depth, -1)
            rsp = ks.expand(depth, B, T, S).reshape(depth, -1)
            rml = km.expand(depth, B, T * S).reshape(depth, -1)
            rt0 = rt * mask0[None, :]
        for i in range(depth):
            live = rates[i] > 0.
            scales.append({'t': rt[i] if live else None, 's': rsp[i] if live else None, 'm': rml[i] if live else None, 't0': rt0[i] if live else mask0})
        return mask0, scales
    for i in range(depth):
        r = rates[i]
        ent = {'t': None, 's': None, 'm': None}
        if forced is not None or (train and r > 0.):
            def draw(kind, shape):
                if forced is not None:
                    if (i, kind) not in forced:
                        return None
                    keep, rate = forced[(i, kind)]
                    return keep.to(dev, torch.float32).reshape(shape) / (1.0 - rate)
                keep = (torch.rand(shape, device=dev) + (1.0 - r)).floor_()
                return keep / (1.0 - r)
            kt = draw('temporal', (B, N))
            if kt is not None:
                rs = torch.ones(B, T, S, dtype=torch.float32, device=dev)
                rs[:, :, 1:] = kt[:, None, :]
                ent['t'] = rs.reshape(-1).contiguous()
            ks = draw('spatial', (B, T))
            if ks is not None:
                ent['s'] = ks[:, :, None].expand(B, T, S).reshape(-1).contiguous()
            km = draw('mlp', (B,))
            if km is not None:
                ent['m'] = km[:, None].expand(B, T * S).reshape(-1).contiguous()
        ent['t0'] = mask0 if ent['t'] is None else ent['t'] * mask0
        scales.append(ent)
    return mask0, scales


def _effective_embeddings(module, g):
    v = module.vit
    pos = v.pos_embed.detach()[0]
    S, T = g['S'], g['T']
    pos_idx = None
    if pos.shape[0] != S:
        n_old = pos.shape[0] - 1
        Pold = int(n_old ** 0.5)
        Hn = S // g['Wp']
        ys = (torch.arange(Hn, device=pos.device).float() * (Pold / Hn)).floor().long().clamp_(max=Pold - 1)
        xs = (torch.arange(g['Wp'], device=pos.device).float() * (Pold / g['Wp'])).floor().long().clamp_(max=Pold - 1)
        grid = (ys[:, None] * Pold + xs[None, :]).reshape(-1) + 1
        pos_idx = torch.cat([torch.zeros(1, dtype=torch.long, device=pos.device), grid])
        pos = pos[pos_idx].contiguous()
    te = v.time_embed.detach()[0]
    time_idx = None
    if te.shape[0] != T:
        time_idx = (torch.arange(T, device=te.device).float() * (te.shape[0] / T)).floor().long().clamp_(max=te.shape[0] - 1)
        te = te[time_idx].contiguous()
    return pos.contiguous(), te.contiguous(), pos_idx, time_idx


def run_forward(module, rgb, qm, params, save, stream=None):
    mode = module.mode
    gmode = module.gemm_mode
    dt = ops.tdtype(mode)
    dev = rgb.device
    B = qm.shape[0]
    g = module.geometry(B) if stream is None else module.geometry(B, T=rgb.shape[2])
    T, S, D, M, P, heads = g['T'], g['S'], g['D'], g['M'], g['P'], g['heads']
    ca = module.causal_attention
    use_cls = ca in (0, 1)
    train = save
    f32 = torch.float32

    def E(*shape, dtype=dt):
        return torch.empty(*shape, dtype=dtype, device=dev)

    opnd = module._operands
    W = lambda p: opnd.weight(mode, p, train)[0]
    mask0, dps = _row_vectors(module, g, module.training)
    sv = {'g': g, 'blocks': [], 'mask0': mask0, 'dps': dps} if save else None

    Kpe = module.input_channels * P * P
    X = E(M, D, dtype=f32)
    Bc = rgb.shape[0]
    Qs = B // Bc
    if Qs > 1:
        Krgb = 3 * P * P
        Wc = W(params[3])
        A_rgb = E(Bc * T * S, Krgb); A_m = E(M, Kpe - Krgb)
        ops.im2col_channels(mode, rgb, P, module.tracker_pretrained, A_rgb)
        ops.im2col_channels(mode, qm, P, False, A_m)
        Xrgb = E(Bc * T * S, D, dtype=f32)
        ops.gemm_nt(gmode, A_rgb, Wc[:, :Krgb], Xrgb, bias=params[4].detach())
        TS = T * S
        for bq in range(B):
            b = bq // Qs
            ops.gemm_nt(gmode, A_m[bq * TS:(bq + 1) * TS], Wc[:, Krgb:], X[bq * TS:(bq + 1) * TS], resid=Xrgb[b * TS:(b + 1) * TS])
        A_pe = (A_rgb, A_m)
    else:
        A_pe = E(M, Kpe)
        ops.im2col(mode, rgb, qm, P, module.tracker_pretrained, A_pe)
        ops.gemm_nt(gmode, A_pe, W(params[3]), X, bias=params[4].detach())
    if stream is None:
        pos, te, pos_idx, time_idx = _effective_embeddings(module, g)
    else:
        pos, te, pos_idx, time_idx = stream.pos, stream.time_rows, None, None
    ops.embed_fwd(X, B, T, S, params[0].detach().reshape(-1), pos, te)
    if save:
        sv.update(A_pe=A_pe, pos_idx=pos_idx, time_idx=time_idx)

    BP, ix = _layout(module)
    joint = module.attention_type != 'divided_space_time'
    fold = fold_on(module)
    amode = gmode if gmode == ops.F32X3 else mode
    shape_attn = ops.attn_shape(amode, B, T, S, D, heads, ca)
    if joint:
        jrows = _joint_rows(module, g, dev)
        Lj = 1 + T * (S - 1)
        shape_joint = ops.attn_shape(amode, B, 1, Lj, D, heads, 0)
    for i in range(module.network_depth):
        q = params[5 + i * BP: 5 + (i + 1) * BP]
        P_ = lambda name, k=0: q[ix[name] + k].detach()
        n1_w, n1_b, qkv_b, proj_b, n2_w, n2_b, fc1_w, fc1_b, fc2_b = P_('n1'), P_('n1', 1), P_('qkv', 1), P_('proj', 1), P_('n2'), P_('n2', 1), P_('fc1'), P_('fc1', 1), P_('fc2', 1)
        dp = dps[i]
        st = {}
        R0 = X
        if joint:
            V = E(M, D); mu1 = E(M, dtype=f32) if save else None; rs1 = E(M, dtype=f32) if save else None
            ops.layernorm_fwd(mode, R0, n1_w, n1_b, V, mu1, rs1)
            QKV2 = E(M, 3 * D)
            ops.gemm_nt(gmode, V, W(q[ix['qkv']]), QKV2, bias=qkv_b)
            QJ = QKV2.index_select(0, jrows)
            OJ = E(B * Lj, D); lse_s = E(B * Lj, heads, dtype=f32) if save else None
            ops.attn_fwd(shape_joint, True, QJ, OJ, lse_s)
            O2 = torch.zeros(M, D, dtype=dt, device=dev)
            O2.index_copy_(0, jrows, OJ)
            rs_s = dp['s']
            R2 = E(M, D, dtype=f32) if save else R0
            ops.gemm_nt(gmode, O2, W(q[ix['proj']]), R2, bias=proj_b, row_scale=rs_s, resid=R0)
            if save:
                st.update(R1=R0, mu1=mu1, rs1=rs1, V=V, QKV_s=QJ, O_s=O2, OJ=OJ, lse_s=lse_s, rs_s=rs_s)
        else:
            tn_w, tn_b, tqkv_b, tproj_b, tfc_b = P_('tn'), P_('tn', 1), P_('tqkv', 1), P_('tproj', 1), P_('tfc', 1)
            U = E(M, D); mu0 = E(M, dtype=f32) if save else None; rs0 = E(M, dtype=f32) if save else None
            ops.layernorm_fwd(mode, R0, tn_w, tn_b, U, mu0, rs0)
            QKV = E(M, 3 * D)
            ops.gemm_nt(gmode, U, W(q[ix['tqkv']]), QKV, bias=tqkv_b)
            O = E(M, D); lse_t = E(M, heads, dtype=f32) if save else None
            if stream is None:
                ops.attn_fwd(shape_attn, False, QKV, O, lse_t)
            else:
                ops.attn_temporal_cached(amode, B, T, S, D, heads, ca, stream.T_total, stream.t0_dev, QKV, stream.k_cache[i], stream.v_cache[i], O)
            R1 = E(M, D, dtype=f32) if save else R0
            if fold:
                Wf, _, bprime = opnd.folded(mode, i, q, ix, train)
                ops.gemm_nt(gmode, O, Wf, R1, bias=bprime, row_scale=dp['t0'], resid=R0, bias2=tfc_b, row_scale2=mask0)
                Pj = None
            else:
                Pj = E(M, D)
                ops.gemm_nt(gmode, O, W(q[ix['tproj']]), Pj, bias=tproj_b, row_scale=dp['t'])
                ops.gemm_nt(gmode, Pj, W(q[ix['tfc']]), R1, bias=tfc_b, row_scale=mask0, resid=R0)
            if save:
                st.update(R0=R0, mu0=mu0, rs0=rs0, U=U, QKV_t=QKV, O_t=O, lse_t=lse_t, Pj=Pj)
            V = E(M, D); mu1 = E(M, dtype=f32) if save else None; rs1 = E(M, dtype=f32) if save else None
            ops.layernorm_fwd(mode, R1, n1_w, n1_b, V, mu1, rs1)
            QKV2 = E(M, 3 * D)
            ops.gemm_nt(gmode, V, W(q[ix['qkv']]), QKV2, bias=qkv_b)
            O2 = E(M, D); lse_s = E(M, heads, dtype=f32) if save else None
            ops.attn_fwd(shape_attn, True, QKV2, O2, lse_s)
            rs_s = dp['s']
            if not use_cls:
                rs_s = mask0 if rs_s is None else rs_s * mask0
            R2 = E(M, D, dtype=f32) if save else R1
            ops.gemm_nt(gmode, O2, W(q[ix['proj']]), R2, bias=proj_b, row_scale=rs_s, resid=R1)
            if use_cls and stream is not None:
                ops.cls_stream(R2, B, T, S, stream.cls_cache[i], stream.t0_dev)
            elif use_cls:
                ops.cls_merge(R2, B, T, S, 1 if ca == 1 else 0)
            if save:
                st.update(R1=R1, mu1=mu1, rs1=rs1, V=V, QKV_s=QKV2, O_s=O2, lse_s=lse_s, rs_s=rs_s)
        Wn = E(M, D); mu2 = E(M, dtype=f32) if save else None; rs2 = E(M, dtype=f32) if save else None
        ops.layernorm_fwd(mode, R2, n2_w, n2_b, Wn, mu2, rs2)
        Hd = fc1_w.shape[0]
        pre = E(M, Hd) if save else None
        H = E(M, Hd)
        ops.gemm_nt(gmode, Wn, W(q[ix['fc1']]), H, bias=fc1_b, act=ACT_GELU_DSAVE if save else ACT_GELU, aux=pre)
        R3 = E(M, D, dtype=f32) if save else R2
        ops.gemm_nt(gmode, H, W(q[ix['fc2']]), R3, bias=fc2_b, row_scale=dp['m'], resid=R2)
        if save:
            st.update(R2=R2, mu2=mu2, rs2=rs2, Wn=Wn, pre=pre, H=H)
            sv['blocks'].append(st)
        X = R3

    nb = 5 + module.network_depth * BP
    norm_w, norm_b, head_w, head_b = params[nb], params[nb + 1], params[nb + 2], params[nb + 3]
    feat32 = X
    if module.norm_embeddings:
        Fm = E(M, D); muf = E(M, dtype=f32) if save else None; rsf = E(M, dtype=f32) if save else None
        ops.layernorm_fwd(mode, X, norm_w.detach(), norm_b.detach(), Fm, muf, rsf)
        if module.flag_channels > 0 and mode != ops.F32:
            feat32 = E(M, D, dtype=f32)
            ops.layernorm_fwd(ops.F32, X, norm_w.detach(), norm_b.detach(), feat32)
        elif mode == ops.F32:
            feat32 = Fm
        if save:
            sv.update(muf=muf, rsf=rsf)
    elif mode == ops.F32:
        Fm = X
    else:
        Fm = E(M, D)
        ops.scale_cast(mode, X, None, Fm)
    Co = module.output_channels
    Pm = E(M, Co * P * P)
    ops.gemm_nt(gmode, Fm, W(head_w), Pm, bias=head_b.detach())
    stp = module.track_map_stride if module.track_map_stride > 1 else 1
    h, w = module.frame_height // stp, module.frame_width // stp
    pooled = E(B * T, Co, h, w, dtype=f32)
    ops.unpatchify_pool_fwd(mode, Pm, B * T, g['Hp'], g['Wp'], P, Co, stp, pooled)
    out_mask = E(B, Co, T, module.frame_height, module.frame_width, dtype=f32)
    bilinear = (module.track_map_resize == 'bilinear') and stp > 1
    ops.upsample_fwd(pooled, B, T, Co, h, w, stp, bilinear, out_mask)
    if module.flag_channels > 0:
        flags = E(B, T, module.flag_channels, dtype=f32)
        ops.flags_fwd(feat32, B * T, S, params[nb + 4].detach(), params[nb + 5].detach(), flags)
    else:
        flags = torch.zeros(0, device=dev)
    if save:
        sv.update(X_final=X, Fm=Fm, feat32=feat32, stp=stp, bilinear=bilinear, h=h, w=w)
    return out_mask, flags, sv


def run_backward(module, sv, params, d_mask, d_flags):
    mode = module.mode
    gmode = module.gemm_mode
    dt = ops.tdtype(mode)
    g = sv['g']
    B, T, S, D, M, P, heads = g['B'], g['T'], g['S'], g['D'], g['M'], g['P'], g['heads']
    dev = sv['X_final'].device
    ca = module.causal_attention
    use_cls = ca in (0, 1)
    f32 = torch.float32
    mask0 = sv['mask0']
    gscale = inv_gscale = None
    ls_mode = getattr(module, 'loss_scale', 'dynamic') if mode == ops.FP16 else None
    if ls_mode == 'dynamic' and module._live_optim() is None and not module._warned_ls:
        import warnings
        module._warned_ls = True
        warnings.warn("precision='fp16' with the dynamic loss scale but no FusedAdamWClip(..., module=net) attached: nothing lowers the scale "
                      "after an overflow or skips the poisoned step -- pass module= to the optimizer or set net.seeker.loss_scale to a number")

    def choose_scale(mask_amax):
        if ls_mode is None:
            return None, None
        if ls_mode == 'dynamic':
            amax = mask_amax if mask_amax is not None else torch.zeros((), dtype=f32, device=dev)
            if d_flags is not None and d_flags.numel():
                amax = torch.maximum(amax, d_flags.detach().abs().amax().to(f32))
            gs = torch.exp2(torch.floor(module.ls_log2 - torch.log2(amax.clamp_min(1e-37)))).clamp(2.0 ** -20, 2.0 ** 60)
        elif float(ls_mode) != 1.0:
            gs = torch.tensor(float(ls_mode), dtype=f32, device=dev)
        else:
            return None, None
        return gs, 1.0 / gs

    def E(*shape, dtype=dt):
        return torch.empty(*shape, dtype=dtype, device=dev)

    opnd = module._operands
    Wt = lambda p: opnd.weight(mode, p, True)[1]
    grads = [None] * len(params)

    defer_unscale = ((module.grad_hook is None or getattr(module.grad_hook, 'active', True) is False) and module._live_optim() is not None
                     and bool(getattr(module, 'persistent_grads', False)) and not getattr(module, '_is_replica', False)
                     and module._defer_unscale)

    def publish(tag, flat):
        if inv_gscale is not None and not defer_unscale:
            flat.mul_(inv_gscale)
        if module.grad_hook is not None:
            module.grad_hook(tag, flat)

    def bucket(indices):
        indices = list(indices)
        total = sum(params[j].numel() for j in indices)
        flat = None
        if getattr(module, 'persistent_grads', False):
            flat = opnd.buffer(('gbuf', indices[0], total, str(dev)), lambda: torch.empty(total, dtype=f32, device=dev))
        if flat is None:
            flat = torch.empty(total, dtype=f32, device=dev)
        off = 0
        for j in indices:
            n = params[j].numel()
            grads[j] = flat[off:off + n].view(params[j].shape)
            off += n
        return flat

    def galloc(idx):
        return grads[idx]

    pending = []

    def linear_bwd(idx_w, dY, Xin, defer=False):
        dW = galloc(idx_w); db = galloc(idx_w + 1)
        if defer:
            pending.append((dY, Xin, dW.reshape(dW.shape[0], -1), db))
        else:
            ops.gemm_tn(gmode, dY, Xin, dW.reshape(dW.shape[0], -1), bias_grad=db)

    tn_group_max = ops.tn_group_max()

    ln_jobs = []

    def flush_pending():
        if pending:
            ops.gemm_tn_grouped(gmode, pending)
            pending.clear()
        if ln_jobs:
            ops.layernorm_fold(ln_jobs)

    BP, ix = _layout(module)
    joint = module.attention_type != 'divided_space_time'
    fold = fold_on(module)
    depth = module.network_depth
    nb = 5 + depth * BP
    Co = module.output_channels
    have_flags = module.flag_channels > 0 and d_flags is not None and d_flags.numel() > 0
    head_idx = ([nb, nb + 1] if module.norm_embeddings else []) + [nb + 2, nb + 3] + ([nb + 4, nb + 5] if have_flags else [])
    group_lo = {}
    hi_ = depth
    for gs in group_sizes(depth):
        for j in range(hi_ - gs, hi_):
            group_lo[j] = hi_ - gs
        hi_ -= gs
    top_lo = group_lo[depth - 1]
    late = set()
    if fold:
        for j in range(depth):
            late.update((5 + j * BP + ix['tproj'], 5 + j * BP + ix['tproj'] + 1, 5 + j * BP + ix['tfc']))
    late_flat = bucket(sorted(late)) if late else None
    blk_idx = lambda lo_, hi_: [j for j in range(5 + lo_ * BP, 5 + hi_ * BP) if j not in late]
    flat_cur = bucket((list(range(0, 5)) if top_lo == 0 else []) + blk_idx(top_lo, depth) + head_idx)
    fold_jobs = []

    def fold_tmp(i):
        return opnd.buffer(('foldtmp', i, str(dev)), lambda: (torch.empty(D, D, dtype=f32, device=dev), torch.empty(D, dtype=f32, device=dev)))

    def finish_fold_group():
        if not fold_jobs:
            return
        nt_, r1_, tn_, gv_ = [], [], [], []
        for (i, tW, tb) in fold_jobs:
            o_ = 5 + i * BP
            wfc, wp, bp = params[o_ + ix['tfc']].detach(), params[o_ + ix['tproj']].detach(), params[o_ + ix['tproj'] + 1].detach()
            nt_.append((tW, wp.t(), grads[o_ + ix['tfc']]))
            r1_.append((tb.view(-1, 1), bp.view(1, -1), grads[o_ + ix['tfc']]))
            tn_.append((wfc.t(), tW, grads[o_ + ix['tproj']]))
            gv_.append((wfc.t(), tb.view(-1, 1), grads[o_ + ix['tproj'] + 1].view(-1, 1)))
        for c0 in range(0, len(nt_), 24):
            ops.sgemm_batched(nt_[c0:c0 + 24]); ops.sgemm_batched(r1_[c0:c0 + 24], accumulate=True)
            ops.sgemm_batched(tn_[c0:c0 + 24]); ops.sgemm_batched(gv_[c0:c0 + 24])
        fold_jobs.clear()

    if d_mask is None:
        d_mask = torch.zeros(B, Co, T, module.frame_height, module.frame_width, dtype=f32, device=dev)
    d_mask = d_mask.to(f32).contiguous()
    dpooled = E(B * T, Co, sv['h'], sv['w'], dtype=f32)
    mask_amax = None
    if ls_mode == 'dynamic' and sv['bilinear'] and sv['stp'] == 4 and sv['h'] > 4 and sv['w'] > 4:
        _, mask_amax = ops.upsample_bwd_amax(d_mask, B, T, Co, sv['h'], sv['w'], sv['stp'], dpooled)
    else:
        if ls_mode == 'dynamic' and d_mask.numel():
            mask_amax = d_mask.abs().amax()
        ops.upsample_bwd(d_mask, B, T, Co, sv['h'], sv['w'], sv['stp'], sv['bilinear'], dpooled)
    gscale, inv_gscale = choose_scale(mask_amax)
    if gscale is not None:
        dpooled.mul_(gscale)
        d_flags = None if d_flags is None else d_flags * gscale
    dPm = E(M, Co * P * P)
    ops.unpatchify_pool_bwd(mode, dpooled, B * T, g['Hp'], g['Wp'], P, Co, sv['stp'], dPm)
    linear_bwd(nb + 2, dPm, sv['Fm'])
    dFeat = E(M, D, dtype=f32)
    ops.gemm_nt(gmode, dPm, Wt(params[nb + 2]), dFeat)
    if module.flag_channels > 0 and have_flags:
        df = d_flags.to(f32).reshape(B * T, -1).contiguous()
        meanf = sv['feat32'].reshape(B * T, S, D)[:, 1:, :].float().mean(dim=1)
        dmean = torch.empty(B * T, D, dtype=f32, device=dev)
        ops.sgemm_batched([(df.t(), meanf, grads[nb + 4])])
        ops.sgemm_batched([(df, params[nb + 4].detach(), dmean)])
        grads[nb + 5].copy_(df.sum(0))
        dFeat.reshape(B * T, S, D)[:, 1:, :] += (dmean / float(S - 1))[:, None, :]
    if module.norm_embeddings:
        dX = E(M, D, dtype=f32)
        ops.layernorm_bwd(ops.F32, dFeat, sv['X_final'], sv['muf'], sv['rsf'], params[nb].detach(), None, dX, galloc(nb), galloc(nb + 1))
    else:
        dX = dFeat
    amode = gmode if gmode == ops.F32X3 else mode
    shape_attn = ops.attn_shape(amode, B, T, S, D, heads, ca)
    if joint:
        jrows = _joint_rows(module, g, dev)
        Lj = 1 + T * (S - 1)
        shape_joint = ops.attn_shape(amode, B, 1, Lj, D, heads, 0)
    dR3 = dX
    G3_next = None
    for i in reversed(range(module.network_depth)):
        o = 5 + i * BP
        q = params[o: o + BP]
        st = sv['blocks'][i]
        dp = sv['dps'][i]
        Hd = q[ix['fc1']].shape[0]
        if i != depth - 1 and group_lo[i] != group_lo[i + 1]:
            lo_ = group_lo[i]
            flat_cur = bucket((list(range(0, 5)) if lo_ == 0 else []) + blk_idx(lo_, i + 1))
        next_scale = (sv['dps'][i - 1]['m'] if i > 0 else mask0)
        if G3_next is not None:
            G3 = G3_next
        else:
            G3 = E(M, D)
            ops.scale_cast(mode, dR3, dp['m'], G3)
        dpre = E(M, Hd)
        ops.gemm_nt(gmode, G3, Wt(q[ix['fc2']]), dpre, act=ACT_MUL_AUX, aux=st['pre'])
        linear_bwd(o + ix['fc2'], G3, st['H'], defer=True)
        dWn = E(M, D)
        ops.gemm_nt(gmode, dpre, Wt(q[ix['fc1']]), dWn)
        linear_bwd(o + ix['fc1'], dpre, st['Wn'], defer=True)
        dR2 = E(M, D, dtype=f32)
        G2 = E(M, D)
        ops.layernorm_bwd(mode, dWn, st['R2'], st['mu2'], st['rs2'], q[ix['n2']].detach(), dR3, dR2, galloc(o + ix['n2']), galloc(o + ix['n2'] + 1),
                          dx_cast=G2, cast_scale=st['rs_s'], defer=ln_jobs)
        del G3, dpre, dWn
        if use_cls and not joint:
            ops.cls_merge(dR2, B, T, S, 1 if ca == 1 else 0, backward=True, cast_mode=mode, cast_out=G2, cast_scale=st['rs_s'])
        dO2 = E(M, D)
        ops.gemm_nt(gmode, G2, Wt(q[ix['proj']]), dO2)
        linear_bwd(o + ix['proj'], G2, st['O_s'], defer=True)
        if joint:
            dQJ = E(B * Lj, 3 * D)
            ops.attn_bwd(shape_joint, True, st['QKV_s'], st['OJ'], dO2.index_select(0, jrows), st['lse_s'], dQJ)
            dQKV2 = torch.zeros(M, 3 * D, dtype=dt, device=dev)
            dQKV2.index_copy_(0, jrows, dQJ)
        else:
            dQKV2 = E(M, 3 * D)
            ops.attn_bwd(shape_attn, True, st['QKV_s'], st['O_s'], dO2, st['lse_s'], dQKV2)
        dV = E(M, D)
        ops.gemm_nt(gmode, dQKV2, Wt(q[ix['qkv']]), dV)
        linear_bwd(o + ix['qkv'], dQKV2, st['V'], defer=True)
        dR1 = E(M, D, dtype=f32)
        G1 = E(M, D)
        if fold:
            ops.layernorm_bwd(mode, dV, st['R1'], st['mu1'], st['rs1'], q[ix['n1']].detach(), dR2, dR1, galloc(o + ix['n1']), galloc(o + ix['n1'] + 1), dx_cast=G1,
                              cast_scale=dp['t0'], colsum_out=galloc(o + ix['tfc'] + 1), colsum_scale=mask0, defer=ln_jobs)
        else:
            ops.layernorm_bwd(mode, dV, st['R1'], st['mu1'], st['rs1'], q[ix['n1']].detach(), dR2, dR1, galloc(o + ix['n1']), galloc(o + ix['n1'] + 1), dx_cast=G1,
                              cast_scale=(next_scale if joint else mask0), defer=ln_jobs)
        del G2, dO2, dQKV2, dV
        if joint:
            G3_next = G1
            dR3 = dR1
        else:
            dO = E(M, D)
            if fold:
                ops.gemm_nt(gmode, G1, opnd.folded(mode, i, q, ix, True)[1], dO)
                tW, tb = fold_tmp(i)
                pending.append((G1, st['O_t'], tW, tb))
                fold_jobs.append((i, tW, tb))
            else:
                dPj = E(M, D)
                ops.gemm_nt(gmode, G1, Wt(q[ix['tfc']]), dPj, row_scale=dp['t'])
                linear_bwd(o + ix['tfc'], G1, st['Pj'], defer=True)
                ops.gemm_nt(gmode, dPj, Wt(q[ix['tproj']]), dO)
                linear_bwd(o + ix['tproj'], dPj, st['O_t'], defer=True)
            dQKV = E(M, 3 * D)
            ops.attn_bwd(shape_attn, False, st['QKV_t'], st['O_t'], dO, st['lse_t'], dQKV)
            dU = E(M, D)
            ops.gemm_nt(gmode, dQKV, Wt(q[ix['tqkv']]), dU)
            linear_bwd(o + ix['tqkv'], dQKV, st['U'], defer=True)
            dR0 = E(M, D, dtype=f32)
            G3_next = E(M, D)
            ops.layernorm_bwd(mode, dU, st['R0'], st['mu0'], st['rs0'], q[ix['tn']].detach(), dR1, dR0, galloc(o + ix['tn']), galloc(o + ix['tn'] + 1),
                              dx_cast=G3_next, cast_scale=next_scale, defer=ln_jobs)
            dR3 = dR0
        if group_lo[i] == i or len(pending) + 8 > tn_group_max:
            flush_pending()
        sv['blocks'][i] = None
        if i > 0 and group_lo[i] == i:
            publish('g%d' % i, flat_cur)

    gX = dR3
    finish_fold_group()
    if late_flat is not None:
        publish('fold', late_flat)
    resized = sv['pos_idx'] is not None or sv['time_idx'] is not None
    dpos_eff = grads[1][0] if sv['pos_idx'] is None else E(S, D, dtype=f32)
    dtime_eff = grads[2][0] if sv['time_idx'] is None else E(T, D, dtype=f32)
    ops.embed_bwd(gX, B, T, S, dpos_eff, dtime_eff)
    grads[0].copy_(dpos_eff[0].reshape(1, 1, D))
    if sv['pos_idx'] is not None:
        grads[1].zero_()
        grads[1][0].index_add_(0, sv['pos_idx'], dpos_eff)
    if sv['time_idx'] is not None:
        grads[2].zero_()
        grads[2][0].index_add_(0, sv['time_idx'], dtime_eff)
    if G3_next is not None:
        Gpe = G3_next
    else:
        Gpe = E(M, D)
        ops.scale_cast(mode, gX, mask0, Gpe)
    dWpe = galloc(3).reshape(D, -1)
    if isinstance(sv['A_pe'], tuple):
        A_rgb, A_m = sv['A_pe']
        Krgb = A_rgb.shape[1]
        Bc = A_rgb.shape[0] // (T * S)
        Gsum = E(Bc * T * S, D)
        ops.scale_cast(mode, gX.reshape(Bc, B // Bc, T * S, D).sum(dim=1).reshape(Bc * T * S, D), mask0[:Bc * T * S], Gsum)
        ops.gemm_tn(gmode, Gsum, A_rgb, dWpe[:, :Krgb])
        ops.gemm_tn(gmode, Gpe, A_m, dWpe[:, Krgb:])
    else:
        ops.gemm_tn(gmode, Gpe, sv['A_pe'], dWpe)
    grads[4].copy_(dtime_eff.sum(0))
    publish('g0', flat_cur)
    module.pending_inv_scale = inv_gscale if defer_unscale else None
    if module.grad_hook is not None:
        if hasattr(module.grad_hook, 'finish'):
            module.grad_hook.finish()
    return grads


class SeekerFunction(torch.autograd.Function):

    @staticmethod
    def forward(ctx, module, rgb, qm, *params):
        need = any(ctx.needs_input_grad[3:])
        ctx.set_materialize_grads(False)
        out_mask, flags, sv = run_forward(module, rgb, qm, params, save=need)
        ctx.module = module
        ctx.sv = sv
        ctx.params = params
        return out_mask, flags

    @staticmethod
    def backward(ctx, d_mask, d_flags):
        if ctx.sv is None:
            raise ops.L.TcowError('backward called on a forward that did not save activations')
        grads = run_backward(ctx.module, ctx.sv, ctx.params, d_mask, d_flags)
        ctx.sv = None
        out = []
        persistent = getattr(ctx.module, 'persistent_grads', False)
        for p, gr, need in zip(ctx.params, grads, ctx.needs_input_grad[3:]):
            if not need or gr is None:
                out.append(None)
                continue
            gr = gr.reshape(p.shape)
            if persistent and (p.grad is None or p.grad.data_ptr() == gr.data_ptr()):
                p.grad = gr
                out.append(None)
            else:
                out.append(gr)
        return (None, None, None, *out)
```

tcow_amd/ops.py:

```python
import ctypes
import threading

import numpy as np
import torch

from . import _lib as L

F32, BF16 = L.TCOW_F32, L.TCOW_BF16
F32X3 = L.TCOW_F32X3
ACT_NONE, ACT_GELU, ACT_DGELU, ACT_GELU_DSAVE, ACT_MUL_AUX = L.ACT_NONE, L.ACT_GELU, L.ACT_DGELU, L.ACT_GELU_DSAVE, L.ACT_MUL_AUX


FP16 = 16


def tdtype(mode):
    return torch.bfloat16 if mode == BF16 else torch.float16 if mode == FP16 else torch.float32


def is16(mode):
    return mode in (BF16, FP16)


def _sel(mode):
    return (L.lib('fp16'), BF16) if mode == FP16 else (L.lib(), mode)


_raw_stream = getattr(torch._C, '_cuda_getCurrentRawStream', None)
_cur_device = getattr(torch._C, '_cuda_getDevice', None)


def _stream():
    if _raw_stream is not None and _cur_device is not None:
        return _raw_stream(_cur_device())
    return torch.cuda.current_stream().cuda_stream


def _p(t):
    return t.data_ptr() if t is not None else None


def _need_cuda(*ts):
    for t in ts:
        if t is not None and not t.is_cuda:
            raise L.TcowError('libtcow_hip kernels need CUDA/HIP tensors (no CPU fallback on this path)')


def gemm_nt(mode, A, W, out, bias=None, row_scale=None, resid=None, act=ACT_NONE, aux=None, tile=0, bias2=None, row_scale2=None):
    _need_cuda(A, W, out)
    M, K = A.shape
    N = W.shape[0]
    lib, dm = _sel(mode)
    a = L.GemmArgs(M, N, K, dm, A.data_ptr(), A.stride(0), W.data_ptr(), W.stride(0), out.data_ptr(), out.stride(0),
                   1 if out.dtype == torch.float32 else 0, _p(bias), _p(row_scale), _p(resid),
                   resid.stride(0) if resid is not None else 0, act, _p(aux), aux.stride(0) if aux is not None else 0, int(tile), _p(bias2), _p(row_scale2))
    L.check(lib.tcow_gemm_nt(_stream(), ctypes.byref(a)), 'tcow_gemm_nt', lib)
    return out


_ws_cache = {}


def workspace(nbytes, device, tag='default'):
    key = (str(device), _stream(), tag, threading.get_ident())
    buf = _ws_cache.get(key)
    if buf is None or buf.numel() < nbytes:
        if buf is None and len(_ws_cache) >= 48:
            alive = {t.ident for t in threading.enumerate()}
            for k in [k for k in _ws_cache if k[3] not in alive]:
                del _ws_cache[k]
        buf = torch.empty(int(nbytes * 1.25) + 1024, dtype=torch.uint8, device=device)
        _ws_cache[key] = buf
    return buf


def gemm_tn(mode, dY, X, dW, bias_grad=None, accumulate=False):
    _need_cuda(dY, X, dW)
    M, N = dY.shape
    K = X.shape[1]
    lib, dm = _sel(mode)
    nbytes = lib.tcow_gemm_tn_workspace_bytes(M, N, K)
    ws = workspace(nbytes, dY.device, 'tn')
    L.check(lib.tcow_gemm_tn(_stream(), dm, M, N, K, dY.data_ptr(), dY.stride(0), X.data_ptr(), X.stride(0), dW.data_ptr(),
                             dW.stride(0), _p(bias_grad), int(accumulate), ws.data_ptr(), ws.numel()), 'tcow_gemm_tn', lib)
    return dW


def tn_group_max():
    return int(L.lib().tcow_gemm_tn_group_max())


def gemm_tn_grouped(mode, problems):
    n = len(problems)
    arr = (L.TnProblem * n)()
    for i, (dY, X, dW, db) in enumerate(problems):
        _need_cuda(dY, X, dW)
        arr[i] = L.TnProblem(dY.shape[0], dY.shape[1], X.shape[1], dY.data_ptr(), dY.stride(0), X.data_ptr(), X.stride(0), dW.data_ptr(), dW.stride(0), _p(db), 0)
    lib, dm = _sel(mode)
    ws = workspace(lib.tcow_gemm_tn_grouped_workspace_bytes(dm, n, arr), problems[0][0].device, 'tn')
    L.check(lib.tcow_gemm_tn_grouped(_stream(), dm, n, arr, ws.data_ptr(), ws.numel()), 'tcow_gemm_tn_grouped', lib)


def sgemm_batched(problems, accumulate=False):
    n = len(problems)
    arr = (L.SGemm * n)()
    for i, (A, B, C) in enumerate(problems):
        _need_cuda(A, B, C)
        M, K = A.shape
        N = B.shape[1]
        assert B.shape[0] == K and C.shape == (M, N) and C.stride(1) == 1 and A.dtype == B.dtype == C.dtype == torch.float32
        arr[i] = L.SGemm(M, N, K, A.data_ptr(), A.stride(0), A.stride(1), B.data_ptr(), B.stride(1), B.stride(0), C.data_ptr(), C.stride(0), 1 if accumulate else 0)
    L.check(L.lib().tcow_sgemm_x3_batched(_stream(), n, arr), 'tcow_sgemm_x3_batched')


def layernorm_fwd(mode, x, gamma, beta, out, mean=None, rstd=None, eps=1e-6):
    rows, D = x.shape
    lib, dm = _sel(mode)
    L.check(lib.tcow_layernorm_fwd(_stream(), dm, rows, D, x.data_ptr(), x.stride(0), gamma.data_ptr(), beta.data_ptr(), eps,
                                       out.data_ptr(), out.stride(0), _p(mean), _p(rstd)), 'tcow_layernorm_fwd', lib)
    return out


def layernorm_bwd(mode, dy, x, mean, rstd, gamma, dres, dx, dgamma=None, dbeta=None, accumulate=False, dx_cast=None, cast_scale=None,
                  colsum_out=None, colsum_scale=None, defer=None):
    rows, D = x.shape
    lib, dm = _sel(mode)
    if defer is not None and dgamma is not None:
        ws = workspace(lib.tcow_layernorm_bwd_workspace_bytes(D), x.device, 'ln_defer%d' % len(defer))
        defer.append((lib, ws, int(lib.tcow_layernorm_bwd_parts(rows, 1 if colsum_out is not None else 0)), D, dgamma, dbeta, colsum_out, bool(accumulate)))
        accumulate = int(accumulate) | 2
    else:
        ws = workspace(lib.tcow_layernorm_bwd_workspace_bytes(D), x.device, 'ln')
    L.check(lib.tcow_layernorm_bwd(_stream(), dm, rows, D, dy.data_ptr(), dy.stride(0), x.data_ptr(), x.stride(0), mean.data_ptr(),
                                   rstd.data_ptr(), gamma.data_ptr(), _p(dres), dres.stride(0) if dres is not None else 0, dx.data_ptr(),
                                   dx.stride(0), _p(dgamma), _p(dbeta), int(accumulate), ws.data_ptr(), ws.numel(),
                                   _p(dx_cast), dx_cast.stride(0) if dx_cast is not None else 0, _p(cast_scale), _p(colsum_scale), _p(colsum_out)), 'tcow_layernorm_bwd', lib)
    return dx


def layernorm_fold(jobs):
    for c0 in range(0, len(jobs), 16):
        chunk = jobs[c0:c0 + 16]
        lib = chunk[0][0]
        arr = (L.LnFoldJob * len(chunk))()
        for i, (_, ws, parts, D, dg, db, cs, acc) in enumerate(chunk):
            arr[i] = L.LnFoldJob(ws.data_ptr(), parts, D, dg.data_ptr(), db.data_ptr(), _p(cs), 1 if acc else 0)
        L.check(lib.tcow_layernorm_fold(_stream(), len(chunk), arr), 'tcow_layernorm_fold', lib)
    jobs.clear()


def attn_shape(mode, B, T, S, D, heads, causal):
    lib, dm = _sel(mode)
    sh = L.AttnShape(B, T, S, D, heads, int(causal), dm)
    sh.tcow_lib = lib
    return sh


def attn_fwd(shape, spatial, qkv, out, lse=None):
    lib = shape.tcow_lib
    fn = lib.tcow_attn_spatial_fwd if spatial else lib.tcow_attn_temporal_fwd
    L.check(fn(_stream(), ctypes.byref(shape), qkv.data_ptr(), out.data_ptr(), _p(lse)), 'tcow_attn_fwd', lib)
    return out


def attn_bwd(shape, spatial, qkv, out, dout, lse, dqkv):
    lib = shape.tcow_lib
    ws = workspace(lib.tcow_attn_bwd_workspace_bytes(ctypes.byref(shape)), qkv.device, 'attn')
    fn = lib.tcow_attn_spatial_bwd if spatial else lib.tcow_attn_temporal_bwd
    L.check(fn(_stream(), ctypes.byref(shape), qkv.data_ptr(), out.data_ptr(), dout.data_ptr(), lse.data_ptr(), dqkv.data_ptr(),
               ws.data_ptr(), ws.numel()), 'tcow_attn_bwd', lib)
    return dqkv


def attn_temporal_cached(mode, B, c, S, D, heads, causal, T_total, t0_dev, qkv, k_cache, v_cache, out):
    _need_cuda(qkv, k_cache, v_cache, out, t0_dev)
    lib, dm = _sel(mode)
    sh = L.AttnShape(B, c, S, D, heads, int(causal), F32 if dm == F32X3 else dm)
    L.check(lib.tcow_attn_temporal_cached_fwd(_stream(), ctypes.byref(sh), int(T_total), t0_dev.data_ptr(), qkv.data_ptr(), k_cache.data_ptr(),
                                              v_cache.data_ptr(), out.data_ptr()), 'tcow_attn_temporal_cached_fwd', lib)
    return out


def cls_stream(x, B, c, S, cls_cache, t0_dev):
    L.check(L.lib().tcow_cls_stream(_stream(), B, c, S, x.shape[1], x.data_ptr(), cls_cache.data_ptr(), t0_dev.data_ptr()), 'tcow_cls_stream')
    return x


def im2col(mode, rgb, query, P, pretrained_norm, out):
    B, _, T, H, W = rgb.shape
    L.check(_sel(mode)[0].tcow_im2col(_stream(), _sel(mode)[1], B, T, H, W, P, rgb.data_ptr(), query.data_ptr(), int(pretrained_norm), out.data_ptr()), 'tcow_im2col', _sel(mode)[0])
    return out


def gather_frames(frames, frame_idx, src_y, src_x):
    _need_cuda(frames, frame_idx, src_y, src_x)
    if frames.element_size() not in (1, 4) or not frames.is_contiguous():
        raise L.TcowError('gather_frames: contiguous tensor of 1- or 4-byte elements expected')
    for t in (frame_idx, src_y, src_x):
        if t.dtype != torch.int32 or not t.is_contiguous():
            raise L.TcowError('gather_frames: index tables must be contiguous int32 tensors')
    C, Tv, H, W = frames.shape
    out = torch.empty(C, frame_idx.numel(), src_y.numel(), src_x.numel(), dtype=frames.dtype, device=frames.device)
    L.check(L.lib().tcow_gather_frames(_stream(), frames.element_size(), C, Tv, H, W, frame_idx.numel(), src_y.numel(), src_x.numel(), frames.data_ptr(),
                                       frame_idx.data_ptr(), src_y.data_ptr(), src_x.data_ptr(), out.data_ptr()), 'tcow_gather_frames')
    return out


def resize_aa(frames, frame_idx, ys, xs, ymin, ysize, wy, ky, xmin, xsize, wx, kx, out_h, out_w):
    _need_cuda(frames, frame_idx, ys, xs, ymin, ysize, wy, xmin, xsize, wx)
    if frames.dtype != torch.float32 or not frames.is_contiguous():
        raise L.TcowError('resize_aa: contiguous f32 frames expected')
    for t, dt in ((frame_idx, torch.int32), (ys, torch.int32), (xs, torch.int32), (ymin, torch.int32), (ysize, torch.int32), (xmin, torch.int32), (xsize, torch.int32),
                  (wy, torch.float32), (wx, torch.float32)):
        if t.dtype != dt or not t.is_contiguous():
            raise L.TcowError('resize_aa: tables must be contiguous int32 / float32 tensors')
    C, Tv, H, W = frames.shape
    out = torch.empty(C, frame_idx.numel(), out_h, out_w, dtype=torch.float32, device=frames.device)
    L.check(L.lib().tcow_resize_aa(_stream(), C, Tv, H, W, frame_idx.numel(), ys.numel(), xs.numel(), out_h, out_w, frames.data_ptr(), frame_idx.data_ptr(), ys.data_ptr(),
                                   xs.data_ptr(), ymin.data_ptr(), ysize.data_ptr(), wy.data_ptr(), int(ky), xmin.data_ptr(), xsize.data_ptr(), wx.data_ptr(), int(kx),
                                   out.data_ptr()), 'tcow_resize_aa')
    return out


def photometric(frames, frame_idx, rect, order, factors, taps, gray):
    import ctypes
    _need_cuda(frames, frame_idx)
    if frames.dtype != torch.float32 or not frames.is_contiguous() or frames.dim() != 4 or frames.shape[0] != 3:
        raise L.TcowError('photometric: contiguous (3, Tv, H, W) f32 frames expected')
    if frame_idx.dtype != torch.int32 or not frame_idx.is_contiguous():
        raise L.TcowError('photometric: frame_idx must be a contiguous int32 tensor')
    _, Tv, H, W = frames.shape
    y0, x0, h, w = (int(v) for v in rect)
    Tc = frame_idx.numel()
    lib = L.lib()
    nb = lib.tcow_photometric_workspace_bytes(Tc)
    ws = torch.empty(max(nb // 4, 1), dtype=torch.float32, device=frames.device)
    out = torch.empty(3, Tc, h, w, dtype=torch.float32, device=frames.device)
    ops_arr = (ctypes.c_int * 4)(*([int(o) for o in order] + [0] * (4 - len(order))))
    taps_arr = (ctypes.c_float * 5)(*([float(t) for t in taps] if taps is not None else [0.0] * 5))
    fb, fc, fs, fh = (float(v) for v in factors)
    L.check(lib.tcow_photometric(_stream(), Tv, H, W, Tc, y0, x0, h, w, frames.data_ptr(), frame_idx.data_ptr(), len(order), ops_arr, fb, fc, fs, fh,
                                 1 if taps is not None else 0, taps_arr, 1 if gray else 0, ws.data_ptr(), nb, out.data_ptr()), 'tcow_photometric')
    return out


def im2col_channels(mode, src, P, normalise, out):
    B, C, T, H, W = src.shape
    L.check(_sel(mode)[0].tcow_im2col_channels(_stream(), _sel(mode)[1], B, T, H, W, P, C, src.data_ptr(), int(normalise), out.data_ptr()), 'tcow_im2col_channels', _sel(mode)[0])
    return out


def embed_fwd(x, B, T, S, cls, pos, time_embed):
    L.check(L.lib().tcow_embed_fwd(_stream(), B, T, S, x.shape[1], x.data_ptr(), cls.data_ptr(), pos.data_ptr(), time_embed.data_ptr()), 'tcow_embed_fwd')
    return x


def embed_bwd(g, B, T, S, dpos, dtime, accumulate=False):
    L.check(L.lib().tcow_embed_bwd(_stream(), B, T, S, g.shape[1], g.data_ptr(), dpos.data_ptr(), dtime.data_ptr(), int(accumulate)), 'tcow_embed_bwd')


def cls_merge(x, B, T, S, mode, backward=False, cast_mode=None, cast_out=None, cast_scale=None):
    if cast_out is not None:
        lib, dm = _sel(cast_mode)
        L.check(lib.tcow_cls_merge_bwd_cast(_stream(), dm, B, T, S, x.shape[1], x.data_ptr(), mode, cast_out.data_ptr(), cast_out.stride(0), _p(cast_scale)), 'tcow_cls_merge_bwd_cast', lib)
        return x
    L.check(L.lib().tcow_cls_merge(_stream(), B, T, S, x.shape[1], x.data_ptr(), mode, int(backward)), 'tcow_cls_merge')
    return x


def unpatchify_pool_fwd(mode, pm, BT, Hp, Wp, P, C, st, pooled):
    L.check(_sel(mode)[0].tcow_unpatchify_pool_fwd(_stream(), _sel(mode)[1], BT, Hp, Wp, P, C, st, pm.data_ptr(), pooled.data_ptr()), 'tcow_unpatchify_pool_fwd', _sel(mode)[0])
    return pooled


def unpatchify_pool_bwd(mode, dpooled, BT, Hp, Wp, P, C, st, dpm):
    L.check(_sel(mode)[0].tcow_unpatchify_pool_bwd(_stream(), _sel(mode)[1], BT, Hp, Wp, P, C, st, dpooled.data_ptr(), dpm.data_ptr()), 'tcow_unpatchify_pool_bwd', _sel(mode)[0])
    return dpm


def upsample_fwd(pooled, B, T, C, h, w, st, bilinear, out):
    L.check(L.lib().tcow_upsample_fwd(_stream(), B, T, C, h, w, st, int(bilinear), pooled.data_ptr(), out.data_ptr()), 'tcow_upsample_fwd')
    return out


def upsample_bwd(dout, B, T, C, h, w, st, bilinear, dpooled):
    L.check(L.lib().tcow_upsample_bwd(_stream(), B, T, C, h, w, st, int(bilinear), dout.data_ptr(), dpooled.data_ptr()), 'tcow_upsample_bwd')
    return dpooled


AMAX_SLOTS = 64


def upsample_bwd_amax(dout, B, T, C, h, w, st, dpooled):
    bits = torch.zeros(AMAX_SLOTS, dtype=torch.int32, device=dout.device)
    L.check(L.lib().tcow_upsample_bwd_amax(_stream(), B, T, C, h, w, st, dout.data_ptr(), dpooled.data_ptr(), bits.data_ptr(), AMAX_SLOTS), 'tcow_upsample_bwd_amax')
    return dpooled, bits.view(torch.float32).amax()


def flags_fwd(x, BT, S, Wf, bf, flags):
    L.check(L.lib().tcow_flags_fwd(_stream(), BT, S, x.shape[1], Wf.shape[0], x.data_ptr(), Wf.data_ptr(), bf.data_ptr(), flags.data_ptr()), 'tcow_flags_fwd')
    return flags


def scale_unless_one(x, scale):
    _need_cuda(x, scale)
    if x.dtype != torch.float32 or not x.is_contiguous() or scale.dtype != torch.float32 or scale.numel() != 1:
        raise L.TcowError('scale_unless_one: a contiguous f32 tensor and a one-element f32 scale')
    L.check(L.lib().tcow_scale_unless_one(_stream(), x.data_ptr(), x.numel(), scale.data_ptr()), 'tcow_scale_unless_one')
    return x


def scale_cast(mode, src, row_scale, dst):
    rows, D = src.shape
    L.check(_sel(mode)[0].tcow_scale_cast(_stream(), _sel(mode)[1], rows, D, src.data_ptr(), src.stride(0), _p(row_scale), dst.data_ptr(), dst.stride(0)), 'tcow_scale_cast', _sel(mode)[0])
    return dst


def droppath_rows(u, keep_p, mask0, B, T, S):
    _need_cuda(u, keep_p, mask0)
    depth = u.shape[0]
    if u.shape[1] != B * (S - 1) + B * T + B or u.dtype != torch.float32 or not u.is_contiguous() or mask0.numel() != B * T * S:
        raise L.TcowError('droppath_rows: u must be contiguous f32 (depth, B*(S-1) + B*T + B), mask0 [B*T*S]')
    out = torch.empty(4, depth, B * T * S, dtype=torch.float32, device=u.device)
    L.check(L.lib().tcow_droppath_rows(_stream(), depth, B, T, S, u.data_ptr(), keep_p.data_ptr(), mask0.data_ptr(), out.data_ptr()), 'tcow_droppath_rows')
    return out


def cast_transpose(mode, W, Wc=None, Wt=None):
    N, K = W.shape
    L.check(_sel(mode)[0].tcow_cast_transpose(_stream(), _sel(mode)[1], N, K, W.data_ptr(), _p(Wc), _p(Wt)), 'tcow_cast_transpose', _sel(mode)[0])


def cast_transpose_batched(mode, table, n, total_tiles):
    L.check(_sel(mode)[0].tcow_cast_transpose_batched(_stream(), _sel(mode)[1], table.data_ptr(), int(n), int(total_tiles)), 'tcow_cast_transpose_batched', _sel(mode)[0])


def mask_loss(logits, target, channel, pixel_w=None, frame_w=None, weighted_aot=False, aot_loss=0.8, topk_frac=1.0,
              loss_weight=1.0, loss_out=None, total=None, dlogits=None, focal=False):
    _need_cuda(logits, target, pixel_w, frame_w, loss_out, total, dlogits)
    BQ, C, T, H, W = logits.shape
    for t in (logits, target, dlogits):
        if t is not None and (t.dtype != torch.float32 or not t.is_contiguous() or t.shape != logits.shape):
            raise L.TcowError('mask_loss: logits / target / dlogits must be contiguous f32 tensors of one shape')
    n_frames, frame_len = BQ * T, H * W
    if pixel_w is not None and (pixel_w.dtype != torch.float32 or not pixel_w.is_contiguous() or pixel_w.numel() != n_frames * frame_len):
        raise L.TcowError('mask_loss: pixel_w must be a contiguous f32 tensor with one weight per pixel')
    if frame_w is not None and (frame_w.dtype != torch.float32 or not frame_w.is_contiguous() or frame_w.numel() != n_frames):
        raise L.TcowError('mask_loss: frame_w must be a contiguous f32 tensor with one weight per frame')
    lib = L.lib()
    nb = lib.tcow_mask_loss_workspace_bytes_for(n_frames, frame_len, float(topk_frac), float(aot_loss))
    ws = workspace(nb, logits.device, 'mask_loss')
    off = channel * T * frame_len * 4
    a = L.MaskLossArgs(n_frames, frame_len, T, logits.data_ptr() + off, C * T * frame_len, target.data_ptr() + off, C * T * frame_len,
                       _p(pixel_w), _p(frame_w), 1 if weighted_aot else 0, float(aot_loss), float(topk_frac), float(loss_weight),
                       loss_out.data_ptr(), _p(total), (dlogits.data_ptr() + off) if dlogits is not None else None,
                       C * T * frame_len, ws.data_ptr(), ws.numel(), 1 if focal else 0)
    L.check(lib.tcow_mask_loss(_stream(), ctypes.byref(a)), 'tcow_mask_loss')
    return loss_out


def mask_loss_channels(logits, target, jobs, aot_loss=0.8, topk_frac=1.0, total=None, dlogits=None, focal=False):
    _need_cuda(logits, target, total, dlogits)
    BQ, C, T, H, W = logits.shape
    for t in (logits, target, dlogits):
        if t is not None and (t.dtype != torch.float32 or not t.is_contiguous() or t.shape != logits.shape):
            raise L.TcowError('mask_loss: logits / target / dlogits must be contiguous f32 tensors of one shape')
    n_frames, frame_len = BQ * T, H * W
    lib = L.lib()
    nb = lib.tcow_mask_loss_workspace_bytes_for(n_frames, frame_len, float(topk_frac), float(aot_loss))
    arr = (L.MaskLossArgs * len(jobs))()
    for i, (channel, pixel_w, frame_w, weighted_aot, loss_weight, loss_out) in enumerate(jobs):
        _need_cuda(pixel_w, frame_w, loss_out)
        if pixel_w is not None and (pixel_w.dtype != torch.float32 or not pixel_w.is_contiguous() or pixel_w.numel() != n_frames * frame_len):
            raise L.TcowError('mask_loss: pixel_w must be a contiguous f32 tensor with one weight per pixel')
        if frame_w is not None and (frame_w.dtype != torch.float32 or not frame_w.is_contiguous() or frame_w.numel() != n_frames):
            raise L.TcowError('mask_loss: frame_w must be a contiguous f32 tensor with one weight per frame')
        ws = workspace(nb, logits.device, 'mask_loss%d' % i)
        off = channel * T * frame_len * 4
        arr[i] = L.MaskLossArgs(n_frames, frame_len, T, logits.data_ptr() + off, C * T * frame_len, target.data_ptr() + off, C * T * frame_len,
                                _p(pixel_w), _p(frame_w), 1 if weighted_aot else 0, float(aot_loss), float(topk_frac), float(loss_weight),
                                loss_out.data_ptr(), _p(total), (dlogits.data_ptr() + off) if dlogits is not None else None,
                                C * T * frame_len, ws.data_ptr(), ws.numel(), 1 if focal else 0)
    L.check(lib.tcow_mask_loss_batch(_stream(), arr, len(jobs)), 'tcow_mask_loss_batch')


def iou_counts(logits, target):
    _need_cuda(logits, target)
    if logits.shape != target.shape or logits.dtype != torch.float32 or target.dtype != torch.float32:
        raise L.TcowError('iou_counts: logits and target must be f32 tensors of one shape')
    lo = logits.contiguous(); tg = target.contiguous()
    frame_len = lo.shape[-1] * lo.shape[-2]
    out = torch.empty(lo.shape[:-2] + (3,), dtype=torch.int32, device=lo.device)
    L.check(L.lib().tcow_iou_counts(_stream(), lo.data_ptr(), tg.data_ptr(), lo.numel() // frame_len, frame_len, out.data_ptr()), 'tcow_iou_counts')
    return out


def build_masks(segm, div_segm, query_idx, front_idx, cont_idx, query_time):
    _need_cuda(segm, div_segm, query_idx, front_idx, cont_idx)
    B, _, T, H, W = segm.shape
    M = div_segm.shape[1]; Q = query_idx.shape[1]
    if segm.dtype != torch.uint8 or div_segm.dtype != torch.uint8 or not segm.is_contiguous() or not div_segm.is_contiguous():
        raise L.TcowError('build_masks: segmentation maps must be contiguous uint8 tensors')
    dev = segm.device
    qm = torch.empty(B, Q, 1, T, H, W, dtype=torch.float32, device=dev); tg = torch.empty(B, Q, 3, T, H, W, dtype=torch.float32, device=dev)
    pt = torch.empty(B, Q, 1, T, H, W, dtype=torch.uint8, device=dev); counts = torch.empty(1 + 2 * Q, dtype=torch.int32, device=dev)
    qi = query_idx.to(torch.int32).contiguous(); fi = front_idx.to(torch.int32).contiguous(); ci = cont_idx.to(torch.int32).contiguous()
    L.check(L.lib().tcow_build_masks(_stream(), B, Q, M, T, H * W, int(query_time), segm.data_ptr(), div_segm.data_ptr(), qi.data_ptr(), fi.data_ptr(),
                                     ci.data_ptr(), qm.data_ptr(), tg.data_ptr(), pt.data_ptr(), counts.data_ptr()), 'tcow_build_masks')
    return qm, tg, pt, counts


def build_query_masks(segm, div_segm, occl_fracs, dag, sel, query_time, front_occl_thres, outer_cont_thres, occluded_weight, occl_cont_zero_weight):
    _need_cuda(segm, div_segm, occl_fracs, dag, sel)
    B, _, T, H, W = segm.shape
    M = div_segm.shape[1]; K = occl_fracs.shape[1]; Q = sel.shape[1]
    if segm.dtype != torch.uint8 or div_segm.dtype != torch.uint8 or not segm.is_contiguous() or not div_segm.is_contiguous():
        raise L.TcowError('build_query_masks: segmentation maps must be contiguous uint8 tensors')
    if tuple(dag.shape) != (B, T, M, M, 3) or tuple(occl_fracs.shape[2:]) != (T, 3) or sel.dtype != torch.int64:
        raise L.TcowError('build_query_masks: occl_fracs (B,K,T,3), dag (B,T,M,M,3) and int64 sel (B,Q) expected')
    dev = segm.device
    of = occl_fracs.to(torch.float32).contiguous(); dg = dag.to(torch.float32).contiguous(); sl = sel.contiguous()
    n = B * Q * T
    qm = torch.empty(B, Q, 1, T, H, W, dtype=torch.float32, device=dev); tg = torch.empty(B, Q, 3, T, H, W, dtype=torch.float32, device=dev)
    pt = torch.empty(B, Q, 1, T, H, W, dtype=torch.uint8, device=dev); counts = torch.empty(1 + 2 * Q, dtype=torch.int32, device=dev)
    idx = torch.empty(B * Q + 2 * n, dtype=torch.int32, device=dev)
    ids = torch.empty(B, Q, T, 2, dtype=torch.uint8, device=dev)
    fl = torch.empty(2, B, Q, T, 3, dtype=torch.float32, device=dev)
    fw = torch.empty(3, B, Q, T, dtype=torch.float32, device=dev)
    f32 = np.float32
    z = f32(occl_cont_zero_weight)
    has_w = f32(f32(1.0 - occl_cont_zero_weight) + z)
    L.check(L.lib().tcow_build_query_masks(_stream(), B, Q, K, M, T, H * W, int(query_time), segm.data_ptr(), div_segm.data_ptr(), of.data_ptr(), dg.data_ptr(),
                                           sl.data_ptr(), float(f32(front_occl_thres)), float(f32(front_occl_thres / 2.0)), float(f32(outer_cont_thres)),
                                           float(f32(float(occluded_weight))), float(z), float(has_w), idx.data_ptr(), ids.data_ptr(), fl[0].data_ptr(),
                                           fl[1].data_ptr(), fw.data_ptr(), qm.data_ptr(), tg.data_ptr(), pt.data_ptr(), counts.data_ptr()),
            'tcow_build_query_masks')
    return {'query_mask': qm, 'target': tg, 'snitch_occl_by_ptr': pt, 'counts': counts, 'ids': ids, 'flags': fl[0], 'sel_occl_fracs': fl[1], 'frame_w': fw,
            'front_idx': idx[B * Q:B * Q + n].view(B, Q, T), 'cont_idx': idx[B * Q + n:].view(B, Q, T)}


def iou_means(counts):
    _need_cuda(counts)
    if counts.dtype != torch.int32 or counts.dim() != 4 or counts.shape[-1] != 3 or not counts.is_contiguous():
        raise L.TcowError('iou_means: contiguous int32 (n_seq, C, T, 3) counts expected')
    n_seq, C, T, _ = counts.shape
    out = torch.empty(12, dtype=torch.float32, device=counts.device)
    cnt = out[6:].view(torch.int32)
    L.check(L.lib().tcow_iou_means(_stream(), counts.data_ptr(), n_seq, C, T, out.data_ptr(), cnt.data_ptr()), 'tcow_iou_means')
    return out[:6], cnt


def snitch_weights(target, snitch_occl_by_ptr, frame_w, pos_count, class_balancing=True, hard_negative_factor=3.0):
    _need_cuda(target, snitch_occl_by_ptr, frame_w, pos_count)
    B, Q, C, T, H, W = target.shape
    if not target.is_contiguous() or not snitch_occl_by_ptr.is_contiguous() or target.dtype != torch.float32 or snitch_occl_by_ptr.dtype != torch.uint8:
        raise L.TcowError('snitch_weights: target must be contiguous f32 and snitch_occl_by_ptr contiguous u8')
    out = torch.empty(B, Q, T, H, W, dtype=torch.float32, device=target.device)
    fw = frame_w.to(torch.float32).contiguous()
    lib = L.lib()
    ws = workspace(lib.tcow_snitch_weights_workspace_bytes(B * Q * T, H, W), target.device, 'snitch_w')
    L.check(lib.tcow_snitch_weights(_stream(), B * Q, T, H, W, target.data_ptr(), C * T * H * W, snitch_occl_by_ptr.data_ptr(), fw.data_ptr(), pos_count.data_ptr(),
                                    1 if class_balancing else 0, float(hard_negative_factor), out.data_ptr(), ws.data_ptr(), ws.numel()), 'tcow_snitch_weights')
    return out
```

Before: 36.98 clips/s.

## Fuse CLS-token copy merge into LayerNorm forward and backward kernels

```diff
diff --git a/include/tcow_hip.h b/include/tcow_hip.h
--- a/include/tcow_hip.h
+++ b/include/tcow_hip.h
@@ -20,7 +20,7 @@
 #define TCOW_ACT_GELU_DSAVE 3
 #define TCOW_ACT_MUL_AUX 4
 
-#define TCOW_ABI_VERSION 11
+#define TCOW_ABI_VERSION 12
 int tcow_version(void);
 const char* tcow_last_error(void);
 
@@ -87,6 +87,13 @@
 } tcow_ln_fold_job;
 int tcow_layernorm_bwd_parts(int rows, int with_colsum);
 int tcow_layernorm_fold(void* stream, int n, const tcow_ln_fold_job* jobs);
+int tcow_layernorm_fwd_cls(void* stream, int dtype, int B, int T, int S, int D, float* x, long ldx, int mode, const float* gamma,
+                           const float* beta, float eps, void* y, long ldy, float* mean, float* rstd);
+int tcow_layernorm_bwd_cls(void* stream, int dtype, int B, int T, int S, int D, int mode, const void* dy, long lddy, const float* x, long ldx,
+                           const float* mean, const float* rstd, const float* gamma, const float* dres, long lddres, float* dx, long lddx,
+                           float* dgamma, float* dbeta, int accumulate, void* workspace, long workspace_bytes, void* dx_cast,
+                           long lddx_cast, const float* cast_row_scale);
+int tcow_layernorm_bwd_cls_parts(int B, int T, int S);
 
 typedef struct {
     int B, T, S;
diff --git a/tcow_amd/_lib.py b/tcow_amd/_lib.py
--- a/tcow_amd/_lib.py
+++ b/tcow_amd/_lib.py
@@ -79,6 +79,9 @@
     'tcow_layernorm_bwd': (_i, [_vp, _i, _i, _i, _vp, _l, _vp, _l, _vp, _vp, _vp, _vp, _l, _vp, _l, _vp, _vp, _i, _vp, _l, _vp, _l, _vp, _vp, _vp]),
     'tcow_layernorm_bwd_parts': (_i, [_i, _i]),
     'tcow_layernorm_fold': (_i, [_vp, _i, _vp]),
+    'tcow_layernorm_fwd_cls': (_i, [_vp, _i, _i, _i, _i, _i, _vp, _l, _i, _vp, _vp, _f, _vp, _l, _vp, _vp]),
+    'tcow_layernorm_bwd_cls': (_i, [_vp, _i, _i, _i, _i, _i, _i, _vp, _l, _vp, _l, _vp, _vp, _vp, _vp, _l, _vp, _l, _vp, _vp, _i, _vp, _l, _vp, _l, _vp]),
+    'tcow_layernorm_bwd_cls_parts': (_i, [_i, _i, _i]),
     'tcow_attn_temporal_fwd': (_i, [_vp, _ash, _vp, _vp, _vp]),
     'tcow_attn_spatial_fwd': (_i, [_vp, _ash, _vp, _vp, _vp]),
     'tcow_attn_bwd_workspace_bytes': (_l, [_ash]),
@@ -127,7 +130,7 @@
 }
 
 
-ABI_VERSION = 11
+ABI_VERSION = 12
 
 
 def _declare(L, tolerant=False):
diff --git a/tcow_amd/csrc/common.h b/tcow_amd/csrc/common.h
--- a/tcow_amd/csrc/common.h
+++ b/tcow_amd/csrc/common.h
@@ -110,6 +110,18 @@
     return v;
 }
 
+__device__ __forceinline__ float4 sum_frames(const float* base, size_t fs, int T_) {
+    float4 a = make_float4(0.f, 0.f, 0.f, 0.f);
+    for (int t0 = 0; t0 < T_; t0 += 8) {
+        float4 v[8];
+#pragma unroll
+        for (int u = 0; u < 8; ++u) v[u] = t0 + u < T_ ? ld4(base + (t0 + u) * fs) : make_float4(0.f, 0.f, 0.f, 0.f);
+#pragma unroll
+        for (int u = 0; u < 8; ++u) { a.x += v[u].x; a.y += v[u].y; a.z += v[u].z; a.w += v[u].w; }
+    }
+    return a;
+}
+
 __host__ __device__ __forceinline__ constexpr int crow32(int r, int hi) { return (r & 3) + 8 * (r >> 2) + 4 * hi; }
 
 void tcow_ensure_lds(const void* kernel, int bytes);
diff --git a/tcow_amd/csrc/elementwise.hip b/tcow_amd/csrc/elementwise.hip
--- a/tcow_amd/csrc/elementwise.hip
+++ b/tcow_amd/csrc/elementwise.hip
@@ -122,17 +122,6 @@
     }
 }
 
-__device__ __forceinline__ float4 sum_frames(const float* base, size_t fs, int T_) {
-    float4 a = make_float4(0.f, 0.f, 0.f, 0.f);
-    for (int t0 = 0; t0 < T_; t0 += 8) {
-        float4 v[8];
-#pragma unroll
-        for (int u = 0; u < 8; ++u) v[u] = t0 + u < T_ ? ld4(base + (t0 + u) * fs) : make_float4(0.f, 0.f, 0.f, 0.f);
-#pragma unroll
-        for (int u = 0; u < 8; ++u) { a.x += v[u].x; a.y += v[u].y; a.z += v[u].z; a.w += v[u].w; }
-    }
-    return a;
-}
 template <typename CT>
 __global__ void cls_merge_kernel(int B, int T_, int S, int D, float* __restrict__ x, int mode, int backward, CT* __restrict__ cast_out, long ldc,
                                  const float* __restrict__ cast_scale) {
diff --git a/tcow_amd/csrc/layernorm.hip b/tcow_amd/csrc/layernorm.hip
--- a/tcow_amd/csrc/layernorm.hip
+++ b/tcow_amd/csrc/layernorm.hip
@@ -6,34 +6,57 @@
 
 constexpr int LN_MAXV = 8;
 
-template <typename T, int NV, bool FULL>
+template <typename T, int NV, bool FULL, bool CLS = false>
 __global__ __launch_bounds__(256) void ln_fwd_kernel(int rows, int D, const float* __restrict__ x, long ldx, const float* __restrict__ gamma,
                                                      const float* __restrict__ beta, float eps, T* __restrict__ y, long ldy,
-                                                     float* __restrict__ mean_out, float* __restrict__ rstd_out) {
+                                                     float* __restrict__ mean_out, float* __restrict__ rstd_out, int cls_S = 0, int cls_T = 0) {
+    auto source = [&](int r, bool* replaced) {
+        *replaced = false;
+        if (!CLS) return r;
+        const int f = r / cls_S;
+        if (r - f * cls_S != 0) return r;
+        const int f0 = f - f % cls_T;
+        *replaced = f != f0;
+        return f0 * cls_S;
+    };
     const int lane = threadIdx.x & 63;
     const int nv = D >> 2;
     const int rstep = gridDim.x * 4;
     int row = blockIdx.x * 4 + (threadIdx.x >> 6);
     if (row >= rows) return;
     float4 g[NV], b[NV], nx[NV];
-#pragma unroll
-    for (int i = 0; i < NV; ++i) {
-        const int c = lane + i * 64;
-        if (FULL || c < nv) { g[i] = ld4(gamma + c * 4); b[i] = ld4(beta + c * 4); nx[i] = ld4(x + (size_t)row * ldx + c * 4); }
+    bool repl_n;
+    {
+        const int src = source(row, &repl_n);
+#pragma unroll
+        for (int i = 0; i < NV; ++i) {
+            const int c = lane + i * 64;
+            if (FULL || c < nv) { g[i] = ld4(gamma + c * 4); b[i] = ld4(beta + c * 4); nx[i] = ld4(x + (size_t)src * ldx + c * 4); }
+        }
     }
     for (; row < rows; row += rstep) {
         float4 v[NV];
         float s = 0.f;
+        const bool repl = repl_n;
 #pragma unroll
         for (int i = 0; i < NV; ++i) {
             const int c = lane + i * 64;
             if (FULL || c < nv) { v[i] = nx[i]; s += (v[i].x + v[i].y) + (v[i].z + v[i].w); }
         }
         if (row + rstep < rows) {
+            const int src = source(row + rstep, &repl_n);
 #pragma unroll
             for (int i = 0; i < NV; ++i) {
                 const int c = lane + i * 64;
-                if (FULL || c < nv) nx[i] = ld4(x + (size_t)(row + rstep) * ldx + c * 4);
+                if (FULL || c < nv) nx[i] = ld4(x + (size_t)src * ldx + c * 4);
+            }
+        }
+        if (CLS && repl) {
+            float* xr = const_cast<float*>(x) + (size_t)row * ldx;
+#pragma unroll
+            for (int i = 0; i < NV; ++i) {
+                const int c = lane + i * 64;
+                if (FULL || c < nv) st4(xr + c * 4, v[i]);
             }
         }
         const float mean = wave_sum(s) / (float)D;
@@ -65,12 +88,13 @@
     }
 }
 
-template <typename T, int NV, bool CSUM, bool FULL>
+template <typename T, int NV, bool CSUM, bool FULL, bool CLS = false>
 __global__ __launch_bounds__(256) void ln_bwd_kernel(int rows, int D, const T* __restrict__ dy, long lddy, const float* __restrict__ x, long ldx,
                                                      const float* __restrict__ mean, const float* __restrict__ rstd,
                                                      const float* __restrict__ gamma, const float* __restrict__ dres, long lddres,
                                                      float* __restrict__ dx, long lddx, float* __restrict__ part ,
-                                                     T* __restrict__ dxc, long lddxc, const float* __restrict__ cscale, const float* __restrict__ sumscale) {
+                                                     T* __restrict__ dxc, long lddxc, const float* __restrict__ cscale, const float* __restrict__ sumscale,
+                                                     int cls_B = 0, int cls_T = 0, int cls_S = 0) {
     constexpr int NP = CSUM ? 3 : 2;
     extern __shared__ __attribute__((aligned(16))) float red[];
     const int lane = threadIdx.x & 63, wave = threadIdx.x >> 6;
@@ -83,8 +107,11 @@
         const int c = lane + i * 64;
         gam[i] = (FULL || c < nv) ? ld4(gamma + c * 4) : gsum[i];
     }
-    const int rstep = gridDim.x * 4;
-    int row = blockIdx.x * 4 + wave;
+    const bool cls_wg = CLS && (int)blockIdx.x < cls_B;
+    const int rstep = !CLS ? (int)gridDim.x * 4 : (cls_wg ? 4 : ((int)gridDim.x - cls_B) * 4);
+    const int nrows = !CLS ? rows : (cls_wg ? cls_T : rows - cls_B * cls_T);
+    int j = !CLS ? blockIdx.x * 4 + wave : (cls_wg ? wave : ((int)blockIdx.x - cls_B) * 4 + wave);
+    auto rowof = [&](int jj) { return !CLS ? jj : (cls_wg ? ((int)blockIdx.x * cls_T + jj) * cls_S : jj + jj / (cls_S - 1) + 1); };
     float4 xn[NV], dn[NV], rn[NV];
     float mu_n = 0.f, rs_n = 0.f;
     auto fetch = [&](int r) {
@@ -109,8 +136,10 @@
             }
         }
     };
-    if (row < rows) fetch(row);
-    for (; row < rows; row += rstep) {
+    int row_n = 0;
+    if (j < nrows) { row_n = rowof(j); fetch(row_n); }
+    for (; j < nrows; j += rstep) {
+        const int row = row_n;
         const float mu = mu_n, rs = rs_n;
         float4 xh[NV], g[NV], rr[NV];
         float s1 = 0.f, s2 = 0.f;
@@ -128,7 +157,7 @@
                 bsum[i].x += d.x; bsum[i].y += d.y; bsum[i].z += d.z; bsum[i].w += d.w;
             }
         }
-        if (row + rstep < rows) fetch(row + rstep);
+        if (j + rstep < nrows) { row_n = rowof(j + rstep); fetch(row_n); }
         const float m1 = wave_sum(s1) / (float)D, m2 = wave_sum(s2) / (float)D;
         float* dxr = dx + (size_t)row * lddx;
         const float cs_row = (dxc && cscale) ? cscale[row] : 1.0f;
@@ -158,6 +187,23 @@
             }
         }
     }
+    if (CLS && cls_wg) {
+        __syncthreads();
+        const size_t fs = (size_t)cls_S * lddx;
+        const size_t r0 = (size_t)blockIdx.x * cls_T * cls_S;
+        for (int c = threadIdx.x * 4; c < D; c += 256 * 4) {
+            float* base = dx + r0 * lddx + c;
+            const float4 a = sum_frames(base, fs, cls_T);
+            const float4 z = make_float4(0.f, 0.f, 0.f, 0.f);
+            st4(base, a);
+            for (int t = 1; t < cls_T; ++t) st4(base + t * fs, z);
+            if (dxc) {
+                const float cs = cscale ? cscale[r0] : 1.0f;
+                st4(dxc + r0 * lddxc + c, make_float4(a.x * cs, a.y * cs, a.z * cs, a.w * cs));
+                for (int t = 1; t < cls_T; ++t) st4(dxc + (r0 + (size_t)t * cls_S) * lddxc + c, z);
+            }
+        }
+    }
     if (!part) return;
 #pragma unroll
     for (int qn = 0; qn < NP; ++qn) {
@@ -184,20 +230,21 @@
 static const int kLnBwdBlocksCsum = 512;
 static const int kLnFwdBlocks = 4096;
 
-extern "C" {
-
-int tcow_layernorm_fwd(void* stream, int dtype, int rows, int D, const float* x, long ldx, const float* gamma, const float* beta, float eps, void* y,
-                       long ldy, float* mean, float* rstd) {
+static int ln_fwd_launch(void* stream, int dtype, int rows, int D, const float* x, long ldx, const float* gamma, const float* beta, float eps, void* y,
+                         long ldy, float* mean, float* rstd, int cls_S, int cls_T) {
     TCOW_CHECK_ARG(rows > 0 && D > 0 && D % 4 == 0 && D <= 64 * 4 * LN_MAXV, "tcow_layernorm_fwd: D=%d must be a multiple of 4 and <= %d", D, 64 * 4 * LN_MAXV);
     TCOW_CHECK_ARG(x && gamma && beta && y && ldx % 4 == 0 && ldy % 4 == 0, "tcow_layernorm_fwd: bad pointers / strides");
+    const bool cls = cls_S > 0;
     int fblocks = cdiv(rows, 4); if (fblocks > kLnFwdBlocks) fblocks = kLnFwdBlocks;
     const dim3 grid(fblocks), block(256);
     if (dtype != TCOW_BF16 && dtype != TCOW_F32) { tcow_set_error("tcow_layernorm_fwd: unknown dtype %d", dtype); return TCOW_ERR_INVALID_ARG; }
     const int nvl = (D / 4 + 63) / 64;
 #define LN_FWD(NVV, FULLV)                                                                                                                               \
     do {                                                                                                                                          \
-        if (dtype == TCOW_BF16) hipLaunchKernelGGL((ln_fwd_kernel<bf16_t, NVV, FULLV>), grid, block, 0, (hipStream_t)stream, rows, D, x, ldx, gamma, beta, eps, (bf16_t*)y, ldy, mean, rstd); \
-        else hipLaunchKernelGGL((ln_fwd_kernel<float, NVV, FULLV>), grid, block, 0, (hipStream_t)stream, rows, D, x, ldx, gamma, beta, eps, (float*)y, ldy, mean, rstd); \
+        if (dtype == TCOW_BF16 && cls) hipLaunchKernelGGL((ln_fwd_kernel<bf16_t, NVV, FULLV, true>), grid, block, 0, (hipStream_t)stream, rows, D, x, ldx, gamma, beta, eps, (bf16_t*)y, ldy, mean, rstd, cls_S, cls_T); \
+        else if (cls) hipLaunchKernelGGL((ln_fwd_kernel<float, NVV, FULLV, true>), grid, block, 0, (hipStream_t)stream, rows, D, x, ldx, gamma, beta, eps, (float*)y, ldy, mean, rstd, cls_S, cls_T); \
+        else if (dtype == TCOW_BF16) hipLaunchKernelGGL((ln_fwd_kernel<bf16_t, NVV, FULLV>), grid, block, 0, (hipStream_t)stream, rows, D, x, ldx, gamma, beta, eps, (bf16_t*)y, ldy, mean, rstd, 0, 0); \
+        else hipLaunchKernelGGL((ln_fwd_kernel<float, NVV, FULLV>), grid, block, 0, (hipStream_t)stream, rows, D, x, ldx, gamma, beta, eps, (float*)y, ldy, mean, rstd, 0, 0); \
     } while (0)
     const bool full = D == 256 * nvl && nvl <= 4;
     if (full) { if (nvl == 1) LN_FWD(1, true); else if (nvl == 2) LN_FWD(2, true); else if (nvl == 3) LN_FWD(3, true); else LN_FWD(4, true); }
@@ -207,12 +254,34 @@
     return TCOW_OK;
 }
 
+extern "C" {
+
+int tcow_layernorm_fwd(void* stream, int dtype, int rows, int D, const float* x, long ldx, const float* gamma, const float* beta, float eps, void* y,
+                       long ldy, float* mean, float* rstd) {
+    return ln_fwd_launch(stream, dtype, rows, D, x, ldx, gamma, beta, eps, y, ldy, mean, rstd, 0, 0);
+}
+
+int tcow_layernorm_fwd_cls(void* stream, int dtype, int B, int T_, int S, int D, float* x, long ldx, int mode, const float* gamma, const float* beta,
+                           float eps, void* y, long ldy, float* mean, float* rstd) {
+    TCOW_CHECK_ARG(B > 0 && T_ > 0 && S > 1 && (long)B * T_ * S < (1L << 31), "tcow_layernorm_fwd_cls: bad B=%d T=%d S=%d", B, T_, S);
+    TCOW_CHECK_ARG(mode == 1, "tcow_layernorm_fwd_cls: only the copy form (mode 1) is fused; mode %d takes tcow_cls_merge + tcow_layernorm_fwd", mode);
+    return ln_fwd_launch(stream, dtype, B * T_ * S, D, x, ldx, gamma, beta, eps, y, ldy, mean, rstd, S, T_);
+}
+
 long tcow_layernorm_bwd_workspace_bytes(int D) { return (long)kLnBwdBlocks * 3 * D * 4; }
 
-int tcow_layernorm_bwd(void* stream, int dtype, int rows, int D, const void* dy, long lddy, const float* x, long ldx, const float* mean,
-                       const float* rstd, const float* gamma, const float* dres, long lddres, float* dx, long lddx, float* dgamma, float* dbeta,
-                       int accumulate, void* workspace, long workspace_bytes, void* dx_cast, long lddx_cast, const float* cast_row_scale,
-                       const float* colsum_row_scale, float* colsum_out) {
+}
+
+static int ln_bwd_cls_blocks(int B, int T_, int S) {
+    int blocks = cdiv((long)B * T_ * (S - 1), 4) + B;
+    if (blocks > kLnBwdBlocks) blocks = kLnBwdBlocks;
+    return blocks;
+}
+
+static int ln_bwd_launch(void* stream, int dtype, int rows, int D, const void* dy, long lddy, const float* x, long ldx, const float* mean,
+                         const float* rstd, const float* gamma, const float* dres, long lddres, float* dx, long lddx, float* dgamma, float* dbeta,
+                         int accumulate, void* workspace, long workspace_bytes, void* dx_cast, long lddx_cast, const float* cast_row_scale,
+                         const float* colsum_row_scale, float* colsum_out, int cls_B, int cls_T, int cls_S) {
     TCOW_CHECK_ARG(rows > 0 && D > 0 && D % 4 == 0 && D <= 64 * 4 * LN_MAXV, "tcow_layernorm_bwd: bad D=%d", D);
     TCOW_CHECK_ARG(dy && x && mean && rstd && gamma && dx, "tcow_layernorm_bwd: null pointer");
     TCOW_CHECK_ARG(!dx_cast || lddx_cast % 4 == 0, "tcow_layernorm_bwd: dx_cast stride must be a multiple of 4");
@@ -222,17 +291,21 @@
     TCOW_CHECK_ARG(!colsum_out || want_param_grads, "tcow_layernorm_bwd: colsum_out rides on the parameter-gradient pass (dgamma / dbeta needed)");
     const bool csum = colsum_out != nullptr;
     const int max_blocks = csum ? kLnBwdBlocksCsum : kLnBwdBlocks;
+    const bool cls = cls_B > 0;
     int blocks = cdiv(rows, 4); if (blocks > max_blocks) blocks = max_blocks;
+    if (cls) blocks = ln_bwd_cls_blocks(cls_B, cls_T, cls_S);
     float* part = want_param_grads ? (float*)workspace : nullptr;
     const size_t lds = want_param_grads ? (size_t)4 * D * 4 : 0;
     if (dtype != TCOW_BF16 && dtype != TCOW_F32) { tcow_set_error("tcow_layernorm_bwd: unknown dtype %d", dtype); return TCOW_ERR_INVALID_ARG; }
     const int nvl = (D / 4 + 63) / 64;
 #define LN_BWD(NVV, FULLV)                                                                                                                               \
     do {                                                                                                                                          \
-        if (dtype == TCOW_BF16 && csum) hipLaunchKernelGGL((ln_bwd_kernel<bf16_t, NVV, true, FULLV>), dim3(blocks), dim3(256), lds, (hipStream_t)stream, rows, D, (const bf16_t*)dy, lddy, x, ldx, mean, rstd, gamma, dres, lddres, dx, lddx, part, (bf16_t*)dx_cast, lddx_cast, cast_row_scale, colsum_row_scale); \
-        else if (dtype == TCOW_BF16) hipLaunchKernelGGL((ln_bwd_kernel<bf16_t, NVV, false, FULLV>), dim3(blocks), dim3(256), lds, (hipStream_t)stream, rows, D, (const bf16_t*)dy, lddy, x, ldx, mean, rstd, gamma, dres, lddres, dx, lddx, part, (bf16_t*)dx_cast, lddx_cast, cast_row_scale, colsum_row_scale); \
-        else if (csum) hipLaunchKernelGGL((ln_bwd_kernel<float, NVV, true, FULLV>), dim3(blocks), dim3(256), lds, (hipStream_t)stream, rows, D, (const float*)dy, lddy, x, ldx, mean, rstd, gamma, dres, lddres, dx, lddx, part, (float*)dx_cast, lddx_cast, cast_row_scale, colsum_row_scale); \
-        else hipLaunchKernelGGL((ln_bwd_kernel<float, NVV, false, FULLV>), dim3(blocks), dim3(256), lds, (hipStream_t)stream, rows, D, (const float*)dy, lddy, x, ldx, mean, rstd, gamma, dres, lddres, dx, lddx, part, (float*)dx_cast, lddx_cast, cast_row_scale, colsum_row_scale); \
+        if (dtype == TCOW_BF16 && cls) hipLaunchKernelGGL((ln_bwd_kernel<bf16_t, NVV, false, FULLV, true>), dim3(blocks), dim3(256), lds, (hipStream_t)stream, rows, D, (const bf16_t*)dy, lddy, x, ldx, mean, rstd, gamma, dres, lddres, dx, lddx, part, (bf16_t*)dx_cast, lddx_cast, cast_row_scale, colsum_row_scale, cls_B, cls_T, cls_S); \
+        else if (cls) hipLaunchKernelGGL((ln_bwd_kernel<float, NVV, false, FULLV, true>), dim3(blocks), dim3(256), lds, (hipStream_t)stream, rows, D, (const float*)dy, lddy, x, ldx, mean, rstd, gamma, dres, lddres, dx, lddx, part, (float*)dx_cast, lddx_cast, cast_row_scale, colsum_row_scale, cls_B, cls_T, cls_S); \
+        else if (dtype == TCOW_BF16 && csum) hipLaunchKernelGGL((ln_bwd_kernel<bf16_t, NVV, true, FULLV>), dim3(blocks), dim3(256), lds, (hipStream_t)stream, rows, D, (const bf16_t*)dy, lddy, x, ldx, mean, rstd, gamma, dres, lddres, dx, lddx, part, (bf16_t*)dx_cast, lddx_cast, cast_row_scale, colsum_row_scale, 0, 0, 0); \
+        else if (dtype == TCOW_BF16) hipLaunchKernelGGL((ln_bwd_kernel<bf16_t, NVV, false, FULLV>), dim3(blocks), dim3(256), lds, (hipStream_t)stream, rows, D, (const bf16_t*)dy, lddy, x, ldx, mean, rstd, gamma, dres, lddres, dx, lddx, part, (bf16_t*)dx_cast, lddx_cast, cast_row_scale, colsum_row_scale, 0, 0, 0); \
+        else if (csum) hipLaunchKernelGGL((ln_bwd_kernel<float, NVV, true, FULLV>), dim3(blocks), dim3(256), lds, (hipStream_t)stream, rows, D, (const float*)dy, lddy, x, ldx, mean, rstd, gamma, dres, lddres, dx, lddx, part, (float*)dx_cast, lddx_cast, cast_row_scale, colsum_row_scale, 0, 0, 0); \
+        else hipLaunchKernelGGL((ln_bwd_kernel<float, NVV, false, FULLV>), dim3(blocks), dim3(256), lds, (hipStream_t)stream, rows, D, (const float*)dy, lddy, x, ldx, mean, rstd, gamma, dres, lddres, dx, lddx, part, (float*)dx_cast, lddx_cast, cast_row_scale, colsum_row_scale, 0, 0, 0); \
     } while (0)
     const bool full = D == 256 * nvl && nvl <= 4;
     if (full) { if (nvl == 1) LN_BWD(1, true); else if (nvl == 2) LN_BWD(2, true); else if (nvl == 3) LN_BWD(3, true); else LN_BWD(4, true); }
@@ -246,6 +319,28 @@
     return TCOW_OK;
 }
 
+extern "C" {
+
+int tcow_layernorm_bwd(void* stream, int dtype, int rows, int D, const void* dy, long lddy, const float* x, long ldx, const float* mean,
+                       const float* rstd, const float* gamma, const float* dres, long lddres, float* dx, long lddx, float* dgamma, float* dbeta,
+                       int accumulate, void* workspace, long workspace_bytes, void* dx_cast, long lddx_cast, const float* cast_row_scale,
+                       const float* colsum_row_scale, float* colsum_out) {
+    return ln_bwd_launch(stream, dtype, rows, D, dy, lddy, x, ldx, mean, rstd, gamma, dres, lddres, dx, lddx, dgamma, dbeta, accumulate, workspace, workspace_bytes,
+                         dx_cast, lddx_cast, cast_row_scale, colsum_row_scale, colsum_out, 0, 0, 0);
+}
+
+int tcow_layernorm_bwd_cls(void* stream, int dtype, int B, int T_, int S, int D, int mode, const void* dy, long lddy, const float* x, long ldx,
+                           const float* mean, const float* rstd, const float* gamma, const float* dres, long lddres, float* dx, long lddx,
+                           float* dgamma, float* dbeta, int accumulate, void* workspace, long workspace_bytes, void* dx_cast, long lddx_cast,
+                           const float* cast_row_scale) {
+    TCOW_CHECK_ARG(B > 0 && B < kLnBwdBlocks && T_ > 0 && S > 1 && (long)B * T_ * S < (1L << 31), "tcow_layernorm_bwd_cls: bad B=%d T=%d S=%d", B, T_, S);
+    TCOW_CHECK_ARG(mode == 1, "tcow_layernorm_bwd_cls: only the copy form (mode 1) is fused; mode %d takes tcow_layernorm_bwd + tcow_cls_merge_bwd_cast", mode);
+    return ln_bwd_launch(stream, dtype, B * T_ * S, D, dy, lddy, x, ldx, mean, rstd, gamma, dres, lddres, dx, lddx, dgamma, dbeta, accumulate, workspace,
+                         workspace_bytes, dx_cast, lddx_cast, cast_row_scale, nullptr, nullptr, B, T_, S);
+}
+
+int tcow_layernorm_bwd_cls_parts(int B, int T_, int S) { return ln_bwd_cls_blocks(B, T_, S); }
+
 int tcow_layernorm_bwd_parts(int rows, int with_colsum) {
     const int max_blocks = with_colsum ? kLnBwdBlocksCsum : kLnBwdBlocks;
     int blocks = cdiv(rows, 4); if (blocks > max_blocks) blocks = max_blocks;
diff --git a/tcow_amd/engine.py b/tcow_amd/engine.py
--- a/tcow_amd/engine.py
+++ b/tcow_amd/engine.py
@@ -194,6 +194,7 @@
         n1_w, n1_b, qkv_b, proj_b, n2_w, n2_b, fc1_w, fc1_b, fc2_b = P_('n1'), P_('n1', 1), P_('qkv', 1), P_('proj', 1), P_('n2'), P_('n2', 1), P_('fc1'), P_('fc1', 1), P_('fc2', 1)
         dp = dps[i]
         st = {}
+        cls_copy = None
         R0 = X
         if joint:
             V = E(M, D); mu1 = E(M, dtype=f32) if save else None; rs1 = E(M, dtype=f32) if save else None
@@ -245,12 +246,14 @@
             ops.gemm_nt(gmode, O2, W(q[ix['proj']]), R2, bias=proj_b, row_scale=rs_s, resid=R1)
             if use_cls and stream is not None:
                 ops.cls_stream(R2, B, T, S, stream.cls_cache[i], stream.t0_dev)
+            elif use_cls and ca != 1:
+                ops.cls_merge(R2, B, T, S, 0)
             elif use_cls:
-                ops.cls_merge(R2, B, T, S, 1 if ca == 1 else 0)
+                cls_copy = (B, T, S)
             if save:
                 st.update(R1=R1, mu1=mu1, rs1=rs1, V=V, QKV_s=QKV2, O_s=O2, lse_s=lse_s, rs_s=rs_s)
         Wn = E(M, D); mu2 = E(M, dtype=f32) if save else None; rs2 = E(M, dtype=f32) if save else None
-        ops.layernorm_fwd(mode, R2, n2_w, n2_b, Wn, mu2, rs2)
+        ops.layernorm_fwd(mode, R2, n2_w, n2_b, Wn, mu2, rs2, cls=cls_copy)
         Hd = fc1_w.shape[0]
         pre = E(M, Hd) if save else None
         H = E(M, Hd)
@@ -495,11 +498,12 @@
         linear_bwd(o + ix['fc1'], dpre, st['Wn'], defer=True)
         dR2 = E(M, D, dtype=f32)
         G2 = E(M, D)
+        cls_copy = (B, T, S) if use_cls and not joint and ca == 1 else None
         ops.layernorm_bwd(mode, dWn, st['R2'], st['mu2'], st['rs2'], q[ix['n2']].detach(), dR3, dR2, galloc(o + ix['n2']), galloc(o + ix['n2'] + 1),
-                          dx_cast=G2, cast_scale=st['rs_s'], defer=ln_jobs)
+                          dx_cast=G2, cast_scale=st['rs_s'], defer=ln_jobs, cls=cls_copy)
         del G3, dpre, dWn
-        if use_cls and not joint:
-            ops.cls_merge(dR2, B, T, S, 1 if ca == 1 else 0, backward=True, cast_mode=mode, cast_out=G2, cast_scale=st['rs_s'])
+        if use_cls and not joint and cls_copy is None:
+            ops.cls_merge(dR2, B, T, S, 0, backward=True, cast_mode=mode, cast_out=G2, cast_scale=st['rs_s'])
         dO2 = E(M, D)
         ops.gemm_nt(gmode, G2, Wt(q[ix['proj']]), dO2)
         linear_bwd(o + ix['proj'], G2, st['O_s'], defer=True)
diff --git a/tcow_amd/ops.py b/tcow_amd/ops.py
--- a/tcow_amd/ops.py
+++ b/tcow_amd/ops.py
@@ -113,24 +113,39 @@
     L.check(L.lib().tcow_sgemm_x3_batched(_stream(), n, arr), 'tcow_sgemm_x3_batched')
 
 
-def layernorm_fwd(mode, x, gamma, beta, out, mean=None, rstd=None, eps=1e-6):
+def layernorm_fwd(mode, x, gamma, beta, out, mean=None, rstd=None, eps=1e-6, cls=None):
     rows, D = x.shape
     lib, dm = _sel(mode)
+    if cls is not None:
+        B, T, S = cls
+        assert rows == B * T * S
+        L.check(lib.tcow_layernorm_fwd_cls(_stream(), dm, B, T, S, D, x.data_ptr(), x.stride(0), 1, gamma.data_ptr(), beta.data_ptr(), eps,
+                                           out.data_ptr(), out.stride(0), _p(mean), _p(rstd)), 'tcow_layernorm_fwd_cls', lib)
+        return out
     L.check(lib.tcow_layernorm_fwd(_stream(), dm, rows, D, x.data_ptr(), x.stride(0), gamma.data_ptr(), beta.data_ptr(), eps,
                                        out.data_ptr(), out.stride(0), _p(mean), _p(rstd)), 'tcow_layernorm_fwd', lib)
     return out
 
 
 def layernorm_bwd(mode, dy, x, mean, rstd, gamma, dres, dx, dgamma=None, dbeta=None, accumulate=False, dx_cast=None, cast_scale=None,
-                  colsum_out=None, colsum_scale=None, defer=None):
+                  colsum_out=None, colsum_scale=None, defer=None, cls=None):
     rows, D = x.shape
     lib, dm = _sel(mode)
     if defer is not None and dgamma is not None:
         ws = workspace(lib.tcow_layernorm_bwd_workspace_bytes(D), x.device, 'ln_defer%d' % len(defer))
-        defer.append((lib, ws, int(lib.tcow_layernorm_bwd_parts(rows, 1 if colsum_out is not None else 0)), D, dgamma, dbeta, colsum_out, bool(accumulate)))
+        parts = lib.tcow_layernorm_bwd_cls_parts(*cls) if cls is not None else lib.tcow_layernorm_bwd_parts(rows, 1 if colsum_out is not None else 0)
+        defer.append((lib, ws, int(parts), D, dgamma, dbeta, colsum_out, bool(accumulate)))
         accumulate = int(accumulate) | 2
     else:
         ws = workspace(lib.tcow_layernorm_bwd_workspace_bytes(D), x.device, 'ln')
+    if cls is not None:
+        B, T, S = cls
+        assert rows == B * T * S and colsum_out is None
+        L.check(lib.tcow_layernorm_bwd_cls(_stream(), dm, B, T, S, D, 1, dy.data_ptr(), dy.stride(0), x.data_ptr(), x.stride(0), mean.data_ptr(),
+                                           rstd.data_ptr(), gamma.data_ptr(), _p(dres), dres.stride(0) if dres is not None else 0, dx.data_ptr(),
+                                           dx.stride(0), _p(dgamma), _p(dbeta), int(accumulate), ws.data_ptr(), ws.numel(),
+                                           _p(dx_cast), dx_cast.stride(0) if dx_cast is not None else 0, _p(cast_scale)), 'tcow_layernorm_bwd_cls', lib)
+        return dx
     L.check(lib.tcow_layernorm_bwd(_stream(), dm, rows, D, dy.data_ptr(), dy.stride(0), x.data_ptr(), x.stride(0), mean.data_ptr(),
                                    rstd.data_ptr(), gamma.data_ptr(), _p(dres), dres.stride(0) if dres is not None else 0, dx.data_ptr(),
                                    dx.stride(0), _p(dgamma), _p(dbeta), int(accumulate), ws.data_ptr(), ws.numel(),
```

After: 37.20 clips/s (median of 6 runs). No clear change (+0.6%).
